# yc015/fully-automated-multi-heartbeat-echocardiography-video-segmentation-and-motion-tracking

Hardware: AMD Instinct MI355X
Metric: 32f×112×112 clips/sec at 1/2/4/8 MI355X; Dice Δ vs CPU ref (higher is better)
Workload: dtype fp32

## Files before the change

### fully-automated-multi-heartbeat-echocardiography-video-segmentation-and-motion-tracking_amd/_lib.py

```python
import ctypes
import os

from .build import LIB_PATH

c_int, c_int64, c_void_p, c_char_p = ctypes.c_int, ctypes.c_int64, ctypes.c_void_p, ctypes.c_char_p
_P = c_void_p

SIGNATURES = {
    "clasfv_last_error": (c_char_p, []),
    "clasfv_version": (c_int, []),
    "clasfv_source_hash": (c_char_p, []),
    "clasfv_create": (c_int, [c_int, ctypes.POINTER(c_void_p)]),
    "clasfv_destroy": (c_int, [_P]),
    "clasfv_param_count": (c_int, [_P]),
    "clasfv_param_info": (c_int, [_P, c_int, ctypes.POINTER(c_char_p), ctypes.POINTER(c_int), ctypes.POINTER(c_int64)]),
    "clasfv_load_param": (c_int, [_P, c_char_p, _P, c_int64]),
    "clasfv_finalize": (c_int, [_P]),
    "clasfv_forward": (c_int, [_P, _P, c_int, c_int, c_int, c_int, _P, _P, _P]),
    "clasfv_workspace_bytes": (c_int64, [_P]),
    "clasfv_set_compute_dtype": (c_int, [_P, c_int]),
    "clasfv_get_compute_dtype": (c_int, [_P]),
    "clasfv_set_kernel_variants": (c_int, [_P, c_int]),
    "clasfv_get_kernel_variants": (c_int, [_P]),
    "clasfv_set_kernel_timing": (c_int, [_P, c_int]),
    "clasfv_kernel_timing": (c_int, [_P, c_int, ctypes.POINTER(c_char_p), ctypes.POINTER(c_int),
                                     ctypes.POINTER(ctypes.c_double), ctypes.POINTER(ctypes.c_double),
                                     ctypes.POINTER(ctypes.c_double)]),
    "clasfv_set_launch_log": (c_int, [_P, c_int]),
    "clasfv_launch_log": (c_int, [_P, c_int, ctypes.POINTER(c_char_p), ctypes.POINTER(c_int64), ctypes.POINTER(c_int),
                                  ctypes.POINTER(c_int)]),
    "clasfv_fill_workspace": (c_int, [_P, c_int, _P]),
    "clasfv_conv_count": (c_int, [_P]),
    "clasfv_conv_info": (c_int, [_P, c_int, ctypes.POINTER(c_char_p), ctypes.POINTER(c_char_p), ctypes.POINTER(c_int),
                                 ctypes.POINTER(c_int), ctypes.POINTER(c_int), ctypes.POINTER(c_int),
                                 ctypes.POINTER(c_int), ctypes.POINTER(c_int), ctypes.POINTER(c_int)]),
    "clasfv_run_conv": (c_int, [_P, c_int, _P, c_int, c_int, c_int, c_int, _P, _P, c_int, c_int, c_int, _P, _P, c_int64,
                                ctypes.POINTER(c_char_p), _P]),
    "clasfv_run_decoder": (c_int, [_P, _P, _P, _P, _P, c_int, c_int, c_int, c_int, _P, _P, _P]),
    "clasfv_build_clips": (c_int, [_P, c_int, c_int, c_int, _P, c_int, c_int, _P, _P]),
    "clasfv_pass_labels": (c_int, [_P, c_int, _P, c_int, c_int, c_int, c_int, c_int, _P, _P]),
    "clasfv_pass_labels_margin": (c_int, [_P, c_int, _P, c_int, c_int, c_int, c_int, c_int, _P, _P]),
    "clasfv_logit_margin": (c_int, [_P, c_int, c_int, c_int, _P, _P]),
    "clasfv_fuse_votes": (c_int, [_P, c_int, c_int, c_int, c_int, c_int, c_int, _P, _P]),
    "clasfv_warp": (c_int, [_P, c_int, c_int, c_int, c_int, _P, c_int64, c_int64, _P, _P]),
    "clasfv_zeroone_workspace_bytes": (c_int64, []),
    "clasfv_zeroone_normalize": (c_int, [_P, c_int64, _P, _P]),
    "clasfv_warp_backward": (c_int, [_P, _P, c_int, c_int, c_int, c_int, _P, c_int64, c_int64, _P, _P, _P]),
    "clasfv_preprocess_video": (c_int, [_P, c_int, c_int, c_int, c_int, c_int, _P, _P]),
    "clasfv_track": (c_int, [_P, c_int, c_int, c_int, c_int, _P, c_int64, c_int64, c_int64, c_int, c_int, c_int, c_int,
                             c_int, _P, _P]),
    "clasfv_lv_geometry": (c_int, [_P, c_int64, c_int, c_int, c_int, ctypes.c_double, ctypes.c_double, _P, _P, _P]),
}

ABI_VERSION = 3
FUSE_MAJORITY, FUSE_SIMPLE, FUSE_STAPLE, FUSE_ITKVOTING = 0, 1, 2, 3
FUSE_FORCE_GENERIC = 0x100
TRACK_BILINEAR, TRACK_NEAREST = 0, 1
TRACK_FORCE_STEPS, TRACK_FORCE_LDS = 0x100, 0x200
TRACK_LDS_MAX_PIXELS, TRACK_LDS_AUTO_PIXELS = 20480, 2304
LV_NPUCKS, LV_STRIDE, LV_MAX_PIXELS = 10, 12, 162816
VARIANTS = {"no_winograd": 1, "no_wino_patch": 2, "winot_reference": 4, "no_c8": 8, "no_stem_bf16": 16,
            "no_patch_bf16": 32, "no_decoder_bf16": 64, "winot_no_ts1": 128, "no_split_k": 256, "no_wino4": 512,
            "no_decoder_x3": 1024, "no_dma_x3": 2048, "no_stem_x3": 4096, "no_wino4w": 8192,
            "no_patch32": 16384, "no_proj_x3": 32768, "no_wino4r": 65536,
            "no_dma_buf": 262144, "w4r_cached_stores": 524288,
            "patch32_cached_stores": 4194304, "no_dma_w": 16777216, "no_twalk": 67108864}
DTYPES = {"fp32": 0, "float32": 0, "bf16": 1, "bfloat16": 1}
_lib = None


def lib_path():
    return LIB_PATH


def load():
    global _lib
    if _lib is not None:
        return _lib
    from . import build as B
    want = B.source_hash()
    have = B.library_hash()
    if have != want:
        import sys
        print(f"clasfv: {LIB_PATH} {'missing' if have is None and not os.path.exists(LIB_PATH) else 'stale'} "
              f"(library source hash {have}, sources {want}): rebuilding", file=sys.stderr)
        B.build()
        if B.library_hash() != want:
            raise RuntimeError(f"{LIB_PATH}: rebuild did not produce a library of the current sources")
    lib = ctypes.CDLL(LIB_PATH)
    for name, (res, args) in SIGNATURES.items():
        fn = getattr(lib, name)
        fn.restype = res
        fn.argtypes = args
    if lib.clasfv_version() != ABI_VERSION:
        raise RuntimeError(f"{LIB_PATH}: ABI version {lib.clasfv_version()}, expected {ABI_VERSION}: rebuild it "
                           f"(python -m clasfv_amd.build --force)")
    got = lib.clasfv_source_hash().decode()
    if got != B.HASH_MARK.decode() + want:
        raise RuntimeError(f"{LIB_PATH}: loaded library reports {got}, sources hash to {want}")
    _lib = lib
    return lib


def check(rc, what=""):
    if rc != 0:
        msg = load().clasfv_last_error()
        raise RuntimeError(f"{what} failed ({rc}): {msg.decode() if msg else ''}")
    return rc


def stream_ptr(stream=None, device=None):
    import torch
    s = stream if stream is not None else torch.cuda.current_stream(device)
    return ctypes.c_void_p(s.cuda_stream)


def ptr(t):
    return ctypes.c_void_p(t.data_ptr())
```

### fully-automated-multi-heartbeat-echocardiography-video-segmentation-and-motion-tracking_amd/build.py

```python
import hashlib
import os
import re
import shutil
import subprocess
import sys

PKG_DIR = os.path.dirname(os.path.abspath(__file__))
REPO_DIR = os.path.dirname(PKG_DIR)
CSRC = os.path.join(PKG_DIR, "csrc")
INCLUDE = os.path.join(REPO_DIR, "include")
LIB_PATH = os.path.join(PKG_DIR, "libclasfv.so")
SOURCES = ["engine.hip", "conv.hip", "conv_patch.hip", "winograd.hip", "winograd2.hip", "winograd4.hip", "winograd4w.hip",
           "winograd_t.hip", "decoder.hip", "plumbing.hip", "twalk.hip", "track.hip", "lvgeom.hip"]
HEADERS = ["common.h", "lvgeom.h", "plumbing.h", "track.h", "warp_math.h", "wino4_common.h"]
ARCH = os.environ.get("CLASFV_OFFLOAD_ARCH", "gfx950")
EXTRA_FLAGS = {"winograd_t.hip": ["-fno-slp-vectorize"]}


def _hipcc():
    for c in (os.environ.get("HIPCC"), "/opt/rocm/bin/hipcc", shutil.which("hipcc")):
        if c and os.path.exists(c):
            return c
    raise RuntimeError("hipcc not found: the CLAS-FV engine needs ROCm's hipcc to build libclasfv.so")


def _inputs():
    files = [os.path.join(CSRC, f) for f in SOURCES + HEADERS]
    files.append(os.path.join(INCLUDE, "clasfv.h"))
    return files


HASH_MARK = b"clasfv-source-hash:"


def source_hash():
    h = hashlib.sha256()
    h.update(repr((ARCH, sorted(EXTRA_FLAGS.items()))).encode())
    for f in _inputs():
        h.update(os.path.basename(f).encode() + b"\0")
        with open(f, "rb") as fh:
            h.update(fh.read())
    return h.hexdigest()[:16]


def library_hash(path=LIB_PATH):
    if not os.path.exists(path):
        return None
    with open(path, "rb") as fh:
        m = re.search(re.escape(HASH_MARK) + rb"([0-9a-f]{16})", fh.read())
    return m.group(1).decode() if m else None


def up_to_date():
    return library_hash() == source_hash()


def build(force=False, verbose=False):
    if not force and up_to_date():
        return LIB_PATH
    import fcntl
    with open(os.path.join(PKG_DIR, "build.lock"), "w") as lock:
        fcntl.flock(lock, fcntl.LOCK_EX)
        if not force and up_to_date():
            return LIB_PATH
        return _build_locked(verbose)


def _build_locked(verbose):
    import tempfile
    from concurrent.futures import ThreadPoolExecutor
    os.makedirs(os.path.join(PKG_DIR, "build_obj"), exist_ok=True)
    objdir = tempfile.mkdtemp(prefix="build-", dir=os.path.join(PKG_DIR, "build_obj"))
    hipcc = _hipcc()
    flags = [f"--offload-arch={ARCH}", "-O3", "-std=c++17", "-fPIC", "-I", INCLUDE]
    digest = source_hash()

    def compile_one(src):
        obj = os.path.join(objdir, os.path.splitext(src)[0] + ".o")
        extra = list(EXTRA_FLAGS.get(src, []))
        if src == "engine.hip":
            extra.append(f'-DCLASFV_SOURCE_HASH="{digest}"')
        cmd = [hipcc] + flags + extra + ["-c", os.path.join(CSRC, src), "-o", obj]
        if verbose:
            print(" ".join(cmd), file=sys.stderr)
        r = subprocess.run(cmd, cwd=CSRC, capture_output=True, text=True)
        if r.returncode != 0:
            raise RuntimeError(f"hipcc failed on {src} ({r.returncode}):\n{r.stderr[-6000:]}")
        return obj

    jobs = max(1, min(len(SOURCES), int(os.environ.get("MAX_JOBS", os.cpu_count() or 4))))
    try:
        with ThreadPoolExecutor(jobs) as ex:
            objs = list(ex.map(compile_one, SOURCES))
        tmp = os.path.join(objdir, "libclasfv.so")
        r = subprocess.run([hipcc, f"--offload-arch={ARCH}", "-shared", "-fPIC", "-o", tmp] + objs,
                           capture_output=True, text=True)
        if r.returncode != 0:
            raise RuntimeError(f"link failed ({r.returncode}):\n{r.stderr[-6000:]}")
        os.replace(tmp, LIB_PATH)
    finally:
        shutil.rmtree(objdir, ignore_errors=True)
    return LIB_PATH


if __name__ == "__main__":
    print(build(force="--force" in sys.argv, verbose=True))
```

### fully-automated-multi-heartbeat-echocardiography-video-segmentation-and-motion-tracking_amd/csrc/common.h

```cpp
#pragma once
#include <hip/hip_runtime.h>
#include <stdint.h>

#include "clasfv.h"

typedef float f32x4 __attribute__((ext_vector_type(4)));
typedef float f32x2 __attribute__((ext_vector_type(2)));

__device__ inline float relu1(float x) { return __int_as_float(max(__float_as_int(x), 0)); }

__device__ inline f32x4 psub4(f32x4 a, f32x4 b) {
  const f32x2 alo = {a[0], a[1]}, ahi = {a[2], a[3]}, blo = {b[0], b[1]}, bhi = {b[2], b[3]};
  f32x2 lo, hi;
  asm("v_pk_add_f32 %0, %1, %2 neg_lo:[0,1] neg_hi:[0,1]" : "=v"(lo) : "v"(alo), "v"(blo));
  asm("v_pk_add_f32 %0, %1, %2 neg_lo:[0,1] neg_hi:[0,1]" : "=v"(hi) : "v"(ahi), "v"(bhi));
  return f32x4{lo[0], lo[1], hi[0], hi[1]};
}


struct FastDiv {
  unsigned m;
  int l;
};
inline FastDiv fast_div(unsigned d) {
  int l = 0;
  while ((1u << l) < d) ++l;
  return FastDiv{(unsigned)(((1ull << 32) * ((1ull << l) - d)) / d + 1), l};
}
__device__ inline int fdiv(int n, FastDiv f) { return (int)((__umulhi((unsigned)n, f.m) + (unsigned)n) >> f.l); }

struct LaunchNote {
  const void* kernel;
  long grid;
  int passes;
};
struct LaunchRing {
  unsigned n;
  LaunchNote e[4];
};
inline thread_local LaunchRing g_launch_ring;
inline void note_launch(const void* kernel, dim3 grid, long passes) {
  LaunchRing& r = g_launch_ring;
  r.e[r.n++ & 3] = LaunchNote{kernel, (long)grid.x * grid.y * grid.z, passes > 1 ? (int)passes : 1};
}
#define CLASFV_LAUNCH_P(passes, kernel, grid, ...)                       \
  do {                                                                   \
    const dim3 launch_grid_ = (grid);                                    \
    note_launch((const void*)(kernel), launch_grid_, (passes));          \
    hipLaunchKernelGGL(kernel, launch_grid_, __VA_ARGS__);               \
  } while (0)
#define CLASFV_LAUNCH(kernel, grid, ...) CLASFV_LAUNCH_P(1, kernel, grid, __VA_ARGS__)

struct ConvParams {
  const void* x;
  const void* w;
  const float* bias;
  const void* res;
  void* y;
  int N, Ti, Hi, Wi, Cin;
  int To, Ho, Wo, Cout;
  int KT, KH, KW, st, sh, sw, pt, ph, pw;
  int K, Kp, M, relu;
  const void* zero;
  const void* x2;
  int Cin2;
  int stem;
  int in_bf16, out_bf16;
  int x_c8, y_c8;
  int vflags, patch_nt;
  float* part;
  int n_split;
};

struct DecTap {
  const float* p;
  int T, H, W;
  float st, sh, sw;
};

struct DecParams {
  DecTap tap[4];
  const float* b1;
  const float* w2;
  const void* w2x3;
  const float* b2;
  const float* wh;
  const float* bh;
  float* seg;
  float* mot;
  int N, T, H, W;
  int bf16;
  int x3;
  void* idx;
};
inline size_t decoder_index_bytes(int T, int H, int W) { return (size_t)4 * (T + H + W) * 16; }

hipError_t launch_conv(const ConvParams& p, int mt, int bn, hipStream_t s);
void conv_pick_tile(int M, int cout_p, int force_nt, int* mt, int* bn);
bool wino_supported(const ConvParams& p);
hipError_t launch_wino(const ConvParams& p, hipStream_t s);
void wino_transform_weights(const double* w, int cout, int cin, int cout_p, int cin_p, float* U);
bool winoq_supported(const ConvParams& p);
hipError_t launch_winoq(const ConvParams& p, hipStream_t s);
bool wino4_supported(const ConvParams& p);
hipError_t launch_wino4(const ConvParams& p, hipStream_t s);
double wino4_exec_gflop(const ConvParams& p);
void wino4_transform_weights(const double* w, int cout, int cin, int cout_p, int cin_p, float* U);
size_t wino4_weight_floats(int cin_p, int cout_p);
bool wino4w_supported(const ConvParams& p);
hipError_t launch_wino4w(const ConvParams& p, hipStream_t s);
double wino4w_exec_gflop(const ConvParams& p);
void wino4w_transform_weights(const double* w, int cout, int cin, int cout_p, int cin_p, float* U);
size_t wino4w_weight_floats(int cin_p, int cout_p);
bool wino4r_supported(const ConvParams& p);
hipError_t launch_wino4r(const ConvParams& p, hipStream_t s);
double wino4r_exec_gflop(const ConvParams& p);
void wino4r_transform_weights(const double* w, int cout, int cin, int cout_p, int cin_p, float* U);
size_t wino4r_weight_floats(int cin_p, int cout_p);
bool winot_supported(const ConvParams& p);
hipError_t launch_winot(const ConvParams& p, hipStream_t s);
bool winot_c8_ok(const ConvParams& p);
hipError_t launch_split_sum(const ConvParams& p, hipStream_t s);
int dma_split_for(const ConvParams& p, int mt);
bool stem_x3_supported(const ConvParams& p);
hipError_t launch_stem_x3(const ConvParams& p, hipStream_t s);
bool dma_x3_supported(const ConvParams& p);
bool dma_w_ok(const ConvParams& p);
int dma_x3_bn(int cout_p);
hipError_t launch_dma_x3(const ConvParams& p, int bn, hipStream_t s);
void dma_x3_weight_image(const float* w, int cout_alloc, int Kp, uint16_t* out);
size_t dma_x3_weight_elems(int cout_alloc, int Kp);
int winot_split_for(const ConvParams& p);
void winot_transform_weights(const double* w, int cout, int cin, int cout_p, int cin_p, float* U);
bool proj_x3_supported(const ConvParams& p);
hipError_t launch_proj_x3(const ConvParams& p, hipStream_t s);
bool patch_bf16_supported(const ConvParams& p);
bool patch32_bf16_supported(const ConvParams& p);
hipError_t launch_patch32_bf16(const ConvParams& p, hipStream_t s);
hipError_t launch_patch_bf16(const ConvParams& p, hipStream_t s);
bool twalk_bf16_supported(const ConvParams& p);
hipError_t launch_twalk_bf16(const ConvParams& p, hipStream_t s);
bool stem_bf16_supported(const ConvParams& p);
hipError_t launch_stem_bf16(const ConvParams& p, hipStream_t s);
hipError_t launch_decoder(const DecParams& p, hipStream_t s);
constexpr int DECODER_X3_ELEMS = 3 * 4096 + 3 * 1024;
void decoder_x3_weights(const float* w2, const float* wh, uint16_t* out);
hipError_t launch_pack_input(const float* x, float* y, int N, int T, int HW, hipStream_t s);
```

### fully-automated-multi-heartbeat-echocardiography-video-segmentation-and-motion-tracking_amd/csrc/decoder.hip

```cpp
#include "common.h"

#include <string.h>

namespace {

constexpr int PIX = 72;
constexpr int TILE_W = 16;
template <int TH>
struct DecGeo {
  static constexpr int NTHR = 32 * TH;
  static constexpr int rows(int i) { return ((TH - 1) >> (i + 1)) + 3; }
  static constexpr int cols(int i) { return (15 >> (i + 1)) + 3; }
  static constexpr int kMaxRows[4] = {rows(0), rows(1), rows(2), rows(3)};
  static constexpr int kMaxCols[4] = {cols(0), cols(1), cols(2), cols(3)};
  static constexpr int kFrames[4] = {1, 2, 2, 2};
  static constexpr int kTapPix[4] = {rows(0) * cols(0), rows(1) * cols(1), rows(2) * cols(2), rows(3) * cols(3)};
  static constexpr int kPixOff[5] = {0, kTapPix[0], kTapPix[0] + kTapPix[1], kTapPix[0] + kTapPix[1] + kTapPix[2],
                                     kTapPix[0] + kTapPix[1] + kTapPix[2] + kTapPix[3]};
  static constexpr int STAGE_FLOATS = kPixOff[4] * PIX;
  static constexpr int ld(int i) { return (kTapPix[i] * 16 + NTHR - 1) / NTHR; }
  static constexpr int kLoads[4] = {ld(0), ld(1), ld(2), ld(3)};
  static constexpr int kLoadOff[4] = {0, ld(0), ld(0) + 2 * ld(1), ld(0) + 2 * ld(1) + 2 * ld(2)};
  static constexpr int kLoadsTotal = ld(0) + 2 * (ld(1) + ld(2) + ld(3));
  static constexpr int kLiveOff[5] = {0, ld(0), ld(0) + ld(1), ld(0) + ld(1) + ld(2), ld(0) + ld(1) + ld(2) + ld(3)};
// ... 189 lines not shown
        for (int mt = 0; mt < 2; ++mt)
          outs[mt] = __builtin_amdgcn_mfma_f32_16x16x4f32(wh[nt][r], acc[mt][nt][r], outs[mt], 0, 0, 0);
  }
#pragma unroll
  for (int mt = 0; mt < 2; ++mt) {
    const int hr = h0 + 2 * wid + mt;
    const f32x4 out = outs[mt];
    if (q < 2) {
      const size_t pix = (size_t)t * HW + (size_t)hr * p.W + (w0 + l16);
#pragma unroll
      for (int r = 0; r < 4; ++r) {
        const int co = 4 * q + r;
        if (co >= 6) continue;
        const float v = out[r];
        if (co < 2)
          p.seg[((size_t)n * 2 + co) * TH + pix] = v;
        else
          p.mot[((size_t)n * 4 + (co - 2)) * TH + pix] = fast_tanh(v);
      }
    }
  }
}

template <int MODE_, int TROWS = 8>
__global__ __launch_bounds__(32 * TROWS) __attribute__((amdgpu_waves_per_eu(((MODE_ & 7) == 4 && !(MODE_ & 64)) ? 4 : 5, ((MODE_ & 7) == 4 && !(MODE_ & 64)) ? 4 : 5))) void decoder_kernel(DecParams p) {
  constexpr int MODE = MODE_ & 7;
  constexpr bool SC = (MODE_ & 8) != 0;
  constexpr bool LIX = (MODE_ & 16) != 0;
  constexpr bool W2S = (MODE_ & 32) != 0;
  using G = DecGeo<TROWS>;
  constexpr int TILE_H = TROWS, NTHR = G::NTHR;
  constexpr int BF = MODE == 1 || MODE == 4;
  extern __shared__ __align__(16) float smem[];
  float* stage = smem;

  const int tid = threadIdx.x, lane = tid & 63;
  const int wid = __builtin_amdgcn_readfirstlane(tid >> 6);
  const int q = lane >> 4, l16 = lane & 15;
  const int tiles_w = p.W / TILE_W, tiles = (p.H / TILE_H) * tiles_w;
  int lt = xcd_swizzle_d(blockIdx.x, gridDim.x);
  const int tile = lt % tiles;
  lt /= tiles;
  const int t = lt % p.T, n = lt / p.T;
  const int h0 = (tile / tiles_w) * TILE_H, w0 = (tile % tiles_w) * TILE_W;


  const DecIdx* tab = reinterpret_cast<const DecIdx*>(p.idx);
  const int per = p.T + p.H + p.W;
  Win win[4];
#pragma unroll
  for (int i = 0; i < 4; ++i) {
    const DecTap& tp = p.tap[i];
    Win w;
    if constexpr (LIX) {
      int a, b;
      float la, lb;
      src_index(tp.st, t, tp.T, a, b, la, lb);
      const bool two = lb > 0.f && b != a && G::kFrames[i] == 2;
      w.t0 = uni(a);
      w.t1 = uni(two ? b : a);
      w.lt0 = unif(two ? la : 1.f);
      w.lt1 = unif(two ? lb : 0.f);
      const int r0 = min((int)floorf(tp.sh * (float)h0), tp.H - 1);
      const int r1 = min((int)floorf(tp.sh * (float)(h0 + TILE_H - 1)) + 1, tp.H - 1);
      const int c0 = min((int)floorf(tp.sw * (float)w0), tp.W - 1);
      const int c1 = min((int)floorf(tp.sw * (float)(w0 + TILE_W - 1)) + 1, tp.W - 1);
      w.r0 = uni(r0);
      w.nr = uni(min(r1 - r0 + 1, G::kMaxRows[i]));
      w.c0 = uni(c0);
      w.nc = uni(min(c1 - c0 + 1, G::kMaxCols[i]));
    } else {
      const DecIdx* ti = tab + i * per;
      const DecIdx ft = ti[t];
      w.t0 = ft.i0;
      w.t1 = ft.i1;
      w.lt0 = ft.l0;
      w.lt1 = ft.l1;
      const int r0 = ti[p.T + h0].i0, r1 = ti[p.T + h0 + TILE_H - 1].i1;
      const int c0 = ti[per - p.W + w0].i0, c1 = ti[per - p.W + w0 + TILE_W - 1].i1;
      w.r0 = r0;
      w.nr = min(r1 - r0 + 1, G::kMaxRows[i]);
      w.c0 = c0;
      w.nc = min(c1 - c0 + 1, G::kMaxCols[i]);
    }
    win[i] = w;
  }
  f32x4 buf[G::kLoadsTotal];
  bool live[G::kLiveOff[4]];
#pragma unroll
  for (int i = 0; i < 4; ++i) {
    const DecTap& tp = p.tap[i];
    const Win& w = win[i];
    const int base0 = (((n * tp.T + w.t0) * tp.H + w.r0) * tp.W + w.c0) * 64;
    const int base1 = base0 + (w.t1 - w.t0) * tp.H * tp.W * 64;
#pragma unroll
    for (int k = 0; k < G::kLoads[i]; ++k) {
      const int e = tid + NTHR * k;
      const int c4 = e & 15, px = e >> 4;
      const int rr = px / G::kMaxCols[i], cc = px - rr * G::kMaxCols[i];
      const bool lv = e < G::kTapPix[i] * 16 && rr < w.nr && cc < w.nc;
      live[G::kLiveOff[i] + k] = lv;
      const int lo = (rr * tp.W + cc) * 64 + c4 * 4;
#pragma unroll
      for (int f = 0; f < G::kFrames[i]; ++f) {
        f32x4& v = buf[G::kLoadOff[i] + k * G::kFrames[i] + f];
        if (lv) v = *reinterpret_cast<const f32x4*>(tp.p + (f ? base1 : base0) + lo);
      }
    }
  }
#pragma unroll
  for (int i = 0; i < 4; ++i) {
    const Win& w = win[i];
    float* dst = stage + G::kPixOff[i] * PIX;
#pragma unroll
    for (int k = 0; k < G::kLoads[i]; ++k) {
      const int e = tid + NTHR * k;
      if (live[G::kLiveOff[i] + k]) {
        f32x4 v = buf[G::kLoadOff[i] + k * G::kFrames[i]];
        if (G::kFrames[i] == 2) {
          const f32x4 v1 = buf[G::kLoadOff[i] + k * G::kFrames[i] + 1];
          if constexpr (SC) {
#pragma unroll
            for (int e = 0; e < 4; ++e) v[e] = fma1(v[e], w.lt0, mul1(v1[e], w.lt1));
          } else {
            v = v * w.lt0 + v1 * w.lt1;
          }
        }
        *reinterpret_cast<f32x4*>(dst + (e >> 4) * PIX + (e & 15) * 4) = v;
      }
    }
  }
  __syncthreads();

  const size_t HW = (size_t)p.H * p.W;
  const size_t TH = (size_t)p.T * HW;
  f32x4 h1[2][4];
#pragma unroll
  for (int mt = 0; mt < 2; ++mt)
#pragma unroll
    for (int c = 0; c < 4; ++c) h1[mt][c] = *reinterpret_cast<const f32x4*>(p.b1 + 16 * c + 4 * q);
  const int hr = h0 + 2 * wid;
#pragma unroll
  for (int i = 0; i < 4; ++i) {
    if constexpr (MODE == 3) {
#pragma unroll
      for (int c = 0; c < 4; ++c) h1[0][c] += *reinterpret_cast<const f32x4*>(stage + G::kPixOff[i] * PIX + 4 * q + 16 * c + l16 * PIX);
      continue;
    }
    const DecTap& tp = p.tap[i];
    const Win& w = win[i];
    int x0, x1, ya0, ya1, yb0, yb1;
    float lx0, lx1, la0, la1, lb0, lb1;
    if constexpr (LIX) {
      src_index(tp.sw, w0 + l16, tp.W, x0, x1, lx0, lx1);
      src_index(tp.sh, hr, tp.H, ya0, ya1, la0, la1);
      src_index(tp.sh, hr + 1, tp.H, yb0, yb1, lb0, lb1);
      ya0 = uni(ya0), ya1 = uni(ya1), yb0 = uni(yb0), yb1 = uni(yb1);
      la0 = unif(la0), la1 = unif(la1), lb0 = unif(lb0), lb1 = unif(lb1);
    } else {
      const DecIdx* ti = tab + i * per;
      const DecIdx cx = ti[per - p.W + w0 + l16];
      const DecIdx ra = ti[p.T + hr], rb = ti[p.T + hr + 1];
      x0 = cx.i0, x1 = cx.i1, lx0 = cx.l0, lx1 = cx.l1;
      ya0 = ra.i0, ya1 = ra.i1, la0 = ra.l0, la1 = ra.l1;
      yb0 = rb.i0, yb1 = rb.i1, lb0 = rb.l0, lb1 = rb.l1;
    }
    const int nrows = yb1 - ya0 + 1;
    const float* fb = stage + G::kPixOff[i] * PIX + 4 * q + (ya0 - w.r0) * G::kMaxCols[i] * PIX;
    const float* c0p = fb + (x0 - w.c0) * PIX;
    const float* c1p = fb + (x1 - w.c0) * PIX;
#pragma unroll
    for (int k = 0; k < 3; ++k) {
      if (k >= nrows) break;
      const bool ta = k == 0 || ya1 - ya0 == k, tb = yb0 - ya0 == k || yb1 - ya0 == k;
      const float wa = (k == 0 ? la0 : 0.f) + (ya1 - ya0 == k ? la1 : 0.f);
      const float wb = (yb0 - ya0 == k ? lb0 : 0.f) + (yb1 - ya0 == k ? lb1 : 0.f);
      const int ro = k * G::kMaxCols[i] * PIX;
      f32x4 hx[4];
      if constexpr (SC) {
#pragma unroll
        for (int c = 0; c < 4; ++c) {
          const f32x4 a0 = *reinterpret_cast<const f32x4*>(c0p + ro + 16 * c), a1 = *reinterpret_cast<const f32x4*>(c1p + ro + 16 * c);
#pragma unroll
          for (int e = 0; e < 4; ++e) hx[c][e] = fma1(a0[e], lx0, mul1(a1[e], lx1));
        }
        if (ta) {
#pragma unroll
          for (int c = 0; c < 4; ++c)
#pragma unroll
            for (int e = 0; e < 4; ++e) h1[0][c][e] = fma1(hx[c][e], wa, h1[0][c][e]);
        }
        if (tb) {
#pragma unroll
          for (int c = 0; c < 4; ++c)
#pragma unroll
            for (int e = 0; e < 4; ++e) h1[1][c][e] = fma1(hx[c][e], wb, h1[1][c][e]);
        }
      } else {
#pragma unroll
        for (int c = 0; c < 4; ++c)
          hx[c] = *reinterpret_cast<const f32x4*>(c0p + ro + 16 * c) * lx0 +
                  *reinterpret_cast<const f32x4*>(c1p + ro + 16 * c) * lx1;
        if (ta) {
#pragma unroll
          for (int c = 0; c < 4; ++c) h1[0][c] += hx[c] * wa;
        }
        if (tb) {
#pragma unroll
          for (int c = 0; c < 4; ++c) h1[1][c] += hx[c] * wb;
        }
      }
      __builtin_amdgcn_sched_barrier(0);
    }
  }
#pragma unroll
  for (int mt = 0; mt < 2; ++mt)
#pragma unroll
    for (int c = 0; c < 4; ++c)
#pragma unroll
      for (int j = 0; j < 4; ++j) h1[mt][c][j] = relu1(h1[mt][c][j]);

  if constexpr (BF) {
    decoder_heads_bf16<MODE == 4, true, W2S>(p, h1, t, n, h0, w0, wid, q, l16);
    return;
  }
  f32x4 acc[2][4], wa[4], wn[4];
#pragma unroll
  for (int c = 0; c < 4; ++c) wa[c] = *reinterpret_cast<const f32x4*>(p.w2 + l16 * 64 + 16 * c + 4 * q);
#pragma unroll
  for (int nt = 0; nt < 4; ++nt) {
    if (nt < 3) {
#pragma unroll
      for (int c = 0; c < 4; ++c)
        wn[c] = *reinterpret_cast<const f32x4*>(p.w2 + ((nt + 1) * 16 + l16) * 64 + 16 * c + 4 * q);
    }
    const f32x4 bb = *reinterpret_cast<const f32x4*>(p.b2 + 16 * nt + 4 * q);
    acc[0][nt] = bb;
    acc[1][nt] = bb;
    if constexpr (MODE == 2) {
#pragma unroll
      for (int mt = 0; mt < 2; ++mt) acc[mt][nt] += wa[nt] * h1[mt][nt];
    } else {
#pragma unroll
      for (int mt = 0; mt < 2; ++mt)
#pragma unroll
        for (int c = 0; c < 4; ++c)
#pragma unroll
          for (int j = 0; j < 4; ++j)
            acc[mt][nt] = __builtin_amdgcn_mfma_f32_16x16x4f32(wa[c][j], h1[mt][c][j], acc[mt][nt], 0, 0, 0);
    }
#pragma unroll
    for (int mt = 0; mt < 2; ++mt)
#pragma unroll
      for (int r = 0; r < 4; ++r) acc[mt][nt][r] = relu1(acc[mt][nt][r]);
#pragma unroll
    for (int c = 0; c < 4; ++c) wa[c] = wn[c];
  }
  f32x4 wh[4];
#pragma unroll
  for (int nt = 0; nt < 4; ++nt) {
    wh[nt] = *reinterpret_cast<const f32x4*>(p.wh + (l16 & 7) * 64 + 16 * nt + 4 * q);
    if (l16 >= 8) wh[nt] = f32x4{0.f, 0.f, 0.f, 0.f};
  }
  f32x4 hb;
#pragma unroll
  for (int r = 0; r < 4; ++r) hb[r] = 4 * q + r < 6 ? p.bh[4 * q + r] : 0.f;
  f32x4 outs[2] = {hb, hb};
  if constexpr (MODE == 2) {
#pragma unroll
    for (int mt = 0; mt < 2; ++mt)
#pragma unroll
      for (int nt = 0; nt < 4; ++nt) outs[mt] += wh[nt] * acc[mt][nt];
  } else {
#pragma unroll
    for (int nt = 0; nt < 4; ++nt)
#pragma unroll
      for (int r = 0; r < 4; ++r)
#pragma unroll
        for (int mt = 0; mt < 2; ++mt)
          outs[mt] = __builtin_amdgcn_mfma_f32_16x16x4f32(wh[nt][r], acc[mt][nt][r], outs[mt], 0, 0, 0);
  }
#pragma unroll
  for (int mt = 0; mt < 2; ++mt) {
    const int hr = h0 + 2 * wid + mt;
    const f32x4 out = outs[mt];
    if (q < 2) {
      const size_t pix = (size_t)t * HW + (size_t)hr * p.W + (w0 + l16);
#pragma unroll
      for (int r = 0; r < 4; ++r) {
        const int co = 4 * q + r;
        if (co >= 6) continue;
        const float v = out[r];
        if (co < 2)
          p.seg[((size_t)n * 2 + co) * TH + pix] = v;
        else
          p.mot[((size_t)n * 4 + (co - 2)) * TH + pix] = fast_tanh(v);
      }
    }
  }
}

}

static hipError_t launch_dec(const DecParams& p, hipStream_t s, int mode, int th = 8) {
  if (p.tap[0].T != p.T) return hipErrorInvalidValue;
  for (int i = 0; i < 4; ++i)
    if ((size_t)p.N * p.tap[i].T * p.tap[i].H * p.tap[i].W * 64 >= ((size_t)1 << 31)) return hipErrorInvalidValue;
  if (p.H % th || p.W % TILE_W) return hipErrorInvalidValue;
  const size_t nb = (size_t)(p.H / th) * (p.W / TILE_W) * p.T * p.N;
  if (nb >= ((size_t)1 << 31)) return hipErrorInvalidValue;
  static_assert(DecGeo<16>::STAGE_FLOATS * 4 <= 64 * 1024, "default dynamic LDS limit");
  const size_t lds = (size_t)(th == 16 ? DecGeo<16>::STAGE_FLOATS : DecGeo<8>::STAGE_FLOATS) * 4;
  void (*k)(DecParams) = nullptr;
  if (th == 8) k = mode == 1 ? decoder_kernel<1> : mode == 4 ? decoder_kernel<4> : mode == 0 ? decoder_kernel<0> : nullptr;
#ifdef CLASFV_KNOCKOUTS
  if (th == 16 && mode < 16) k = mode == 1 ? decoder_kernel<1, 16> : mode == 4 ? decoder_kernel<4, 16> : decoder_kernel<0, 16>;
  if (mode == 2) k = th == 16 ? decoder_kernel<2, 16> : decoder_kernel<2>;
  if (mode == 3) k = th == 16 ? decoder_kernel<3, 16> : decoder_kernel<3>;
  if (mode == 12) k = th == 16 ? decoder_kernel<12, 16> : decoder_kernel<12>;
  if (mode == 9) k = th == 16 ? decoder_kernel<9, 16> : decoder_kernel<9>;
  if (th == 8 && mode == 1 + 16 + 32) k = decoder_kernel<1 + 16 + 32>;
  if (th == 8 && mode == 4 + 16) k = decoder_kernel<4 + 16>;
  if (th == 8 && mode == 0 + 16) k = decoder_kernel<0 + 16>;
  if (th == 8 && mode == 1 + 16) k = decoder_kernel<1 + 16>;
  if (th == 8 && mode == 1 + 32) k = decoder_kernel<1 + 32>;
  if (th == 8 && mode == 4 + 64) k = decoder_kernel<4 + 64>;
#endif
  if (!k) return hipErrorInvalidValue;
  if (!(mode & 16)) {
    if (!p.idx) return hipErrorInvalidValue;
    const int ne = 4 * (p.T + p.H + p.W);
    CLASFV_LAUNCH(decoder_index_kernel, dim3((unsigned)((ne + 255) / 256)), dim3(256), 0, s, p);
  }
  CLASFV_LAUNCH(k, dim3((unsigned)nb), dim3(32 * th), lds, s, p);
  return hipGetLastError();
}

void decoder_x3_weights(const float* w2, const float* wh, uint16_t* out) {
  auto put = [&](double r, size_t i0, size_t stride) {
    for (int pc = 0; pc < 3; ++pc) {
      float f = (float)r;
      uint32_t u;
      memcpy(&u, &f, 4);
      const uint16_t b = (uint16_t)((u + 0x7fffu + ((u >> 16) & 1u)) >> 16);
      const uint32_t ub = (uint32_t)b << 16;
      float fb;
      memcpy(&fb, &ub, 4);
      out[i0 + pc * stride] = b;
      r -= fb;
    }
  };
  for (int nt = 0; nt < 4; ++nt)
    for (int kb = 0; kb < 2; ++kb)
      for (int l = 0; l < 16; ++l)
        for (int q = 0; q < 4; ++q)
          for (int e = 0; e < 8; ++e)
            put(w2[(16 * nt + l) * 64 + 32 * kb + 4 * q + (e < 4 ? e : 12 + e)],
                ((((size_t)nt * 2 + kb) * 16 + l) * 4 + q) * 8 + e, 4096);
  for (int kb = 0; kb < 2; ++kb)
    for (int l = 0; l < 16; ++l)
      for (int q = 0; q < 4; ++q)
        for (int e = 0; e < 8; ++e)
          put(l < 8 ? wh[l * 64 + 32 * kb + 4 * q + (e < 4 ? e : 12 + e)] : 0.0,
              3 * 4096 + (((size_t)kb * 16 + l) * 4 + q) * 8 + e, 1024);
}

hipError_t launch_decoder(const DecParams& p, hipStream_t s) {
  if ((p.x3 || p.bf16) && !p.w2x3) return hipErrorInvalidValue;
  const int mode = p.bf16 ? 1 : p.x3 ? 4 : 0;
  return launch_dec(p, s, mode, 8);
}

#ifdef CLASFV_KNOCKOUTS
hipError_t launch_decoder_ko(const DecParams& p, hipStream_t s, int ko) {
  const int m = ko & 15;
  const int base = m == 2 || m == 3 ? m : (p.bf16 ? 1 : p.x3 ? 4 : 0);
  int mode = (ko & 32) && (base == 1 || base == 4) ? base + 8 : base;
  if (ko & 64) mode += 16;
  if ((ko & 128) && base == 1) mode += 32;
  if ((ko & 256) && base == 4) mode += 64;
  return launch_dec(p, s, mode, (ko & 16) ? 16 : 8);
}
#endif
```

### fully-automated-multi-heartbeat-echocardiography-video-segmentation-and-motion-tracking_amd/csrc/engine.hip

```cpp
#include <cxxabi.h>
#include <math.h>
#include <stdio.h>
#include <stdlib.h>
#include <string.h>

#include <string>
#include <unordered_map>
#include <vector>

#include "clasfv.h"
#include "common.h"
#include "lvgeom.h"
#include "plumbing.h"
#include "track.h"

namespace {

thread_local std::string g_err;

int fail(int code, const std::string& msg) {
  g_err = msg;
  return code;
}

#define HIP_TRY(expr)                                                                        \
  do {                                                                                       \
    hipError_t _e = (expr);                                                                  \
    if (_e != hipSuccess) return fail(CLASFV_EHIP, std::string(#expr) + ": " + hipGetErrorString(_e)); \
  } while (0)

constexpr double kBnEps = 1e-5;

struct Param {
  std::string name;
  std::vector<int64_t> shape;
  std::vector<float> data;
  bool loaded = false;
  int64_t numel() const {
    int64_t n = 1;
    for (auto d : shape) n *= d;
    return n;
  }
};

int round_up(int x, int m) { return (x + m - 1) / m * m; }

int pad_channels(int c, bool bf16) {
  if (c == 3) return 4;
  const int step = bf16 ? 32 : 16;
  int cp = round_up(c, step);
  auto ok = [](int cp_) {
    for (int nt : {9, 8, 6, 5, 4, 3})
      if ((cp_ / 16) % nt == 0) return true;
    return false;
  };
  while (!ok(cp)) cp += step;
  return cp;
}

enum Role { STEM_S, STEM_T, SP1, TP1, SP2, TP2, DS, PROJ };

struct Conv {
  Role role;
  std::string w, bn;
  int cin, cout, cin_p, cout_p;
  int kt, kh, kw, st, sh, sw, pt, ph, pw;
  int K, Kp, cout_alloc;
  int cin2 = 0;
  int stem = 0, in_bf16 = 0, out_bf16 = 0;
  void* dw = nullptr;
  float* db = nullptr;
  void* dwino = nullptr;
  void* dwino4 = nullptr;
  void* dwino4w = nullptr;
  void* dwino4r = nullptr;
  void* dwinot = nullptr;
  void* dws16 = nullptr;
  void* dx3 = nullptr;
};

using ConvImage = void* Conv::*;
constexpr ConvImage kConvImages[] = {&Conv::dw,      &Conv::dwino,  &Conv::dwino4, &Conv::dwino4w,
                                     &Conv::dwino4r, &Conv::dwinot, &Conv::dws16,  &Conv::dx3};

void free_conv_images(Conv& c) {
  for (ConvImage img : kConvImages) {
    (void)hipFree(c.*img);
    c.*img = nullptr;
  }
  (void)hipFree(c.db);
  c.db = nullptr;
}

bool use_winot(const Conv& c, bool bf16, int vflags) {
  if (vflags & CLASFV_VARIANT_NO_WINOGRAD) return false;
  return !bf16 && (c.role == STEM_T || c.role == TP1 || c.role == TP2) && c.kt == 3 && c.kh == 1 && c.kw == 1 &&
         c.st == 1 && c.cin_p % 8 == 0 && c.cout_p % 64 == 0;
}

bool use_wino(const Conv& c, bool bf16, int vflags) {
  if (vflags & CLASFV_VARIANT_NO_WINOGRAD) return false;
  return !bf16 && (c.role == SP1 || c.role == SP2) && c.kt == 1 && c.kh == 3 && c.kw == 3 && c.sh == 1 &&
         c.sw == 1 && c.cin_p % 16 == 0 && c.cout_p % 48 == 0;
}

struct VariantSwitch {
  int bit;
  const char* env;
  bool zero_form;
};
constexpr VariantSwitch kVariants[] = {
    {CLASFV_VARIANT_NO_WINOGRAD, "CLASFV_WINOGRAD", true},
    {CLASFV_VARIANT_NO_WINO_PATCH, "CLASFV_NO_WINO_PATCH", false},
    {CLASFV_VARIANT_WINOT_REFERENCE, "CLASFV_WINOT_REFERENCE", false},
    {CLASFV_VARIANT_NO_C8, "CLASFV_NO_C8", false},
    {CLASFV_VARIANT_NO_STEM_BF16, "CLASFV_NO_STEM_BF16", false},
    {CLASFV_VARIANT_NO_PATCH_BF16, "CLASFV_NO_PATCH_BF16", false},
    {CLASFV_VARIANT_NO_DECODER_BF16, "CLASFV_NO_DECODER_BF16", false},
    {CLASFV_VARIANT_WINOT_NO_TS1, "CLASFV_WINOT_TS1", true},
    {CLASFV_VARIANT_NO_SPLIT_K, "CLASFV_NO_SPLIT_K", false},
    {CLASFV_VARIANT_NO_WINO4, "CLASFV_NO_WINO4", false},
    {CLASFV_VARIANT_NO_DECODER_X3, "CLASFV_NO_DECODER_X3", false},
    {CLASFV_VARIANT_NO_DMA_X3, "CLASFV_NO_DMA_X3", false},
    {CLASFV_VARIANT_NO_STEM_X3, "CLASFV_NO_STEM_X3", false},
    {CLASFV_VARIANT_NO_WINO4W, "CLASFV_NO_WINO4W", false},
    {CLASFV_VARIANT_NO_PATCH32, "CLASFV_NO_PATCH32", false},
    {CLASFV_VARIANT_NO_PROJ_X3, "CLASFV_NO_PROJ_X3", false},
    {CLASFV_VARIANT_NO_WINO4R, "CLASFV_NO_WINO4R", false},
    {CLASFV_VARIANT_NO_DMA_BUF, "CLASFV_NO_DMA_BUF", false},
    {CLASFV_VARIANT_W4R_CACHED_STORES, "CLASFV_W4R_CACHED_STORES", false},
    {CLASFV_VARIANT_PATCH32_CACHED_STORES, "CLASFV_PATCH32_CACHED_STORES", false},
    {CLASFV_VARIANT_NO_DMA_W, "CLASFV_NO_DMA_W", false},
    {CLASFV_VARIANT_NO_TWALK, "CLASFV_NO_TWALK", false},
};

int env_variants() {
  int f = 0;
  for (const VariantSwitch& v : kVariants) {
    const char* e = getenv(v.env);
    if (e && (!v.zero_form || e[0] == '0')) f |= v.bit;
  }
  return f;
}

constexpr int variant_mask() {
  int m = 0;
  for (const VariantSwitch& v : kVariants) m |= v.bit;
  return m;
}
constexpr int kVariantMask = variant_mask();

int env_int(const char* name) {
  const char* e = getenv(name);
  return e ? atoi(e) : 0;
}

void layout_conv(Conv& c, bool bf16) {
  c.stem = (c.role == STEM_S);
  c.in_bf16 = bf16 && !c.stem;
  c.out_bf16 = bf16 && c.role != PROJ;
  c.cin_p = pad_channels(c.cin, bf16);
  c.cout_p = c.role == PROJ ? c.cout : pad_channels(c.cout, bf16);
  c.K = c.kt * c.kh * c.kw * c.cin_p + c.cin2;
  c.Kp = round_up(c.K, c.in_bf16 ? 32 : 16);
  c.cout_alloc = c.cout_p;
}

Conv make_conv(Role role, const std::string& w, const std::string& bn, int cin, int cout, int kt, int kh, int kw,
               int st, int sh, int sw, int pt, int ph, int pw) {
  Conv c;
  c.role = role;
  c.w = w;
  c.bn = bn;
  c.cin = cin;
  c.cout = cout;
  c.kt = kt, c.kh = kh, c.kw = kw, c.st = st, c.sh = sh, c.sw = sw, c.pt = pt, c.ph = ph, c.pw = pw;
  layout_conv(c, false);
  return c;
}

int midplanes(int i, int o) { return (i * o * 27) / (i * 9 + 3 * o); }

struct Tuning {
  int vflags = 0, conv_nt = 0, patch_nt = 0;
};

}

struct clasfv_engine {
  int device = 0;
  std::vector<Param> params;
  std::unordered_map<std::string, int> index;
  std::vector<Conv> convs;
  Conv proj[5];
  float *b1 = nullptr, *w2 = nullptr, *b2 = nullptr, *wh = nullptr, *bh = nullptr;
  void* w2x3 = nullptr;
  bool ready = false;
  int dtype = CLASFV_DTYPE_FP32;
  Tuning tune;
  float* zero = nullptr;
  struct Ctx {
    hipStream_t stream = nullptr;
    char* arena = nullptr;
    size_t arena_bytes = 0;
    hipStream_t side = nullptr;
    hipEvent_t ev_fork = nullptr, ev_join = nullptr;
    uint64_t last_use = 0;
  };
  std::vector<Ctx*> ctxs;
  uint64_t ctx_clock = 0;
  bool ktime = false;
  std::vector<hipEvent_t> evs;
  int nev = 0;
  struct Rec {
    const char* name;
    double gflop;
    double xgflop;
    int e0, e1;
  };
  std::vector<Rec> recs;
  bool llog = false;
  struct LogRec {
    const char* label;
    long grid;
    int passes, conv;
  };
  std::vector<LogRec> log;
  std::unordered_map<const void*, std::string> labels;
};

namespace {

void add_param(clasfv_engine* e, const std::string& name, std::vector<int64_t> shape) {
  Param p;
  p.name = name;
  p.shape = std::move(shape);
  e->index[name] = (int)e->params.size();
  e->params.push_back(std::move(p));
}

void add_bn(clasfv_engine* e, const std::string& pre, int c) {
  add_param(e, pre + ".weight", {c});
  add_param(e, pre + ".bias", {c});
  add_param(e, pre + ".running_mean", {c});
  add_param(e, pre + ".running_var", {c});
  add_param(e, pre + ".num_batches_tracked", {});
}

void build_plan(clasfv_engine* e) {
  const std::string R = "r2plus1d_model.";
  auto reg = [&](const Conv& c) {
    add_param(e, c.w + ".weight", {c.cout, c.cin, c.kt, c.kh, c.kw});
    add_bn(e, c.bn, c.cout);
    e->convs.push_back(c);
  };
  reg(make_conv(STEM_S, R + "stem.0", R + "stem.1", 3, 45, 1, 7, 7, 1, 2, 2, 0, 3, 3));
  reg(make_conv(STEM_T, R + "stem.3", R + "stem.4", 45, 64, 3, 1, 1, 1, 1, 1, 1, 0, 0));
  int inplanes = 64;
  const int planes_l[4] = {64, 128, 256, 512}, stride_l[4] = {1, 2, 2, 2};
  for (int li = 0; li < 4; ++li) {
    const int planes = planes_l[li], stride = stride_l[li];
    for (int b = 0; b < 2; ++b) {
      const int st = b == 0 ? stride : 1;
      const int cin1 = b == 0 ? inplanes : planes;
      const int mid = midplanes(cin1, planes);
      const std::string pre = R + "layer" + std::to_string(li + 1) + "." + std::to_string(b) + ".";
      reg(make_conv(SP1, pre + "conv1.0.0", pre + "conv1.0.1", cin1, mid, 1, 3, 3, 1, st, st, 0, 1, 1));
      reg(make_conv(TP1, pre + "conv1.0.3", pre + "conv1.1", mid, planes, 3, 1, 1, st, 1, 1, 1, 0, 0));
      reg(make_conv(SP2, pre + "conv2.0.0", pre + "conv2.0.1", planes, mid, 1, 3, 3, 1, 1, 1, 0, 1, 1));
      reg(make_conv(TP2, pre + "conv2.0.3", pre + "conv2.1", mid, planes, 3, 1, 1, 1, 1, 1, 1, 0, 0));
      if (b == 0 && (stride != 1 || inplanes != planes))
        reg(make_conv(DS, pre + "downsample.0", pre + "downsample.1", inplanes, planes, 1, 1, 1, stride, stride,
                      stride, 0, 0, 0));
    }
    inplanes = planes;
  }
  add_param(e, R + "fc.weight", {400, 512});
  add_param(e, R + "fc.bias", {400});
  add_param(e, "comb_1_layer.weight", {64, 1024, 1, 1, 1});
  add_param(e, "comb_1_layer.bias", {64});
  add_bn(e, "comb_batch_norm_1", 64);
  add_param(e, "comb_2_layer.weight", {64, 64, 1, 1, 1});
  add_param(e, "comb_2_layer.bias", {64});
  add_bn(e, "comb_batch_norm_2", 64);
  add_param(e, "motion_head.weight", {4, 64, 1, 1, 1});
  add_param(e, "motion_head.bias", {4});
  add_param(e, "segmentation_head.weight", {2, 64, 1, 1, 1});
  add_param(e, "segmentation_head.bias", {2});
  const int tap_c[5] = {64, 64, 128, 256, 512};
  for (int i = 0; i < 5; ++i) e->proj[i] = make_conv(PROJ, "", "", tap_c[i], 64, 1, 1, 1, 1, 1, 1, 0, 0, 0);
  e->proj[0].cin2 = 64;
  layout_conv(e->proj[0], false);
}

const std::vector<float>& P(clasfv_engine* e, const std::string& n) { return e->params[e->index.at(n)].data; }

void bn_scale_shift(clasfv_engine* e, const std::string& bn, int c, std::vector<double>& s, std::vector<double>& t) {
  const auto& g = P(e, bn + ".weight");
  const auto& b = P(e, bn + ".bias");
  const auto& m = P(e, bn + ".running_mean");
  const auto& v = P(e, bn + ".running_var");
  s.resize(c);
  t.resize(c);
  for (int i = 0; i < c; ++i) {
    s[i] = (double)g[i] / sqrt((double)v[i] + kBnEps);
    t[i] = (double)b[i] - (double)m[i] * s[i];
  }
}

template <class T>
int upload(const std::vector<float>& h, T** d) {
  HIP_TRY(hipMalloc(d, h.size() * sizeof(float)));
  HIP_TRY(hipMemcpy(*d, h.data(), h.size() * sizeof(float), hipMemcpyHostToDevice));
  return CLASFV_OK;
}

uint16_t to_bf16(float f) {
  uint32_t u;
  memcpy(&u, &f, 4);
  u += 0x7FFF + ((u >> 16) & 1);
  return (uint16_t)(u >> 16);
}

int upload_bf16(const std::vector<float>& h, void** d) {
  std::vector<uint16_t> b(h.size());
  for (size_t i = 0; i < h.size(); ++i) b[i] = to_bf16(h[i]);
  HIP_TRY(hipMalloc(d, b.size() * sizeof(uint16_t)));
  HIP_TRY(hipMemcpy(*d, b.data(), b.size() * sizeof(uint16_t), hipMemcpyHostToDevice));
  return CLASFV_OK;
}

template <class F>
int upload_conv(Conv& c, F wsrc, const std::vector<double>& scale, const std::vector<double>& shift, bool has_bias) {
  std::vector<float> w((size_t)c.cout_alloc * c.Kp, 0.f);
  const int taps = c.kt * c.kh * c.kw;
  for (int o = 0; o < c.cout; ++o)
    for (int tap = 0; tap < taps; ++tap)
      for (int ci = 0; ci < c.cin; ++ci)
        w[(size_t)o * c.Kp + (size_t)tap * c.cin_p + ci] = (float)((double)wsrc(o, ci, tap) * scale[o]);
  int rc = c.in_bf16 ? upload_bf16(w, &c.dw) : upload(w, &c.dw);
  if (rc) return rc;
  if (!c.in_bf16 && !c.stem && c.Kp % 16 == 0) {
    std::vector<uint16_t> x3(dma_x3_weight_elems(c.cout_alloc, c.Kp));
    dma_x3_weight_image(w.data(), c.cout_alloc, c.Kp, x3.data());
    HIP_TRY(hipMalloc(&c.dx3, x3.size() * sizeof(uint16_t)));
    HIP_TRY(hipMemcpy(c.dx3, x3.data(), x3.size() * sizeof(uint16_t), hipMemcpyHostToDevice));
  }
  if (has_bias) {
    std::vector<float> b(c.cout_alloc, 0.f);
    for (int o = 0; o < c.cout; ++o) b[o] = (float)shift[o];
    rc = upload(b, &c.db);
  }
  return rc;
}

std::vector<double> folded_weights(const Conv& c, const std::vector<float>& w, const std::vector<double>& s, int taps) {
  const size_t per_o = (size_t)c.cin * taps;
  std::vector<double> wf((size_t)c.cout * per_o);
  for (int o = 0; o < c.cout; ++o)
    for (size_t i = 0; i < per_o; ++i) wf[o * per_o + i] = (double)w[o * per_o + i] * s[o];
  return wf;
}

int upload_wino_images(Conv& c, const std::vector<float>& w, const std::vector<double>& s) {
  const std::vector<double> wf = folded_weights(c, w, s, 9);
  int rc;
  std::vector<float> u((size_t)16 * c.cin_p * c.cout_p);
  wino_transform_weights(wf.data(), c.cout, c.cin, c.cout_p, c.cin_p, u.data());
  if ((rc = upload(u, &c.dwino))) return rc;
  if (c.cout_p % 48 == 0 && c.cin_p % 8 == 0) {
    std::vector<float> u4(wino4_weight_floats(c.cin_p, c.cout_p));
    wino4_transform_weights(wf.data(), c.cout, c.cin, c.cout_p, c.cin_p, u4.data());
    if ((rc = upload(u4, &c.dwino4))) return rc;
  }
  if (c.cin_p % 8 == 0 && wino4w_weight_floats(c.cin_p, c.cout_p)) {
    std::vector<float> uw(wino4w_weight_floats(c.cin_p, c.cout_p));
    wino4w_transform_weights(wf.data(), c.cout, c.cin, c.cout_p, c.cin_p, uw.data());
    if ((rc = upload(uw, &c.dwino4w))) return rc;
  }
  if (c.cin_p % 8 == 0 && wino4r_weight_floats(c.cin_p, c.cout_p)) {
    std::vector<float> ur(wino4r_weight_floats(c.cin_p, c.cout_p));
    wino4r_transform_weights(wf.data(), c.cout, c.cin, c.cout_p, c.cin_p, ur.data());
    if ((rc = upload(ur, &c.dwino4r))) return rc;
  }
  return CLASFV_OK;
}

int upload_winot_image(Conv& c, const std::vector<float>& w, const std::vector<double>& s) {
  const std::vector<double> wf = folded_weights(c, w, s, 3);
  std::vector<float> u((size_t)6 * c.cin_p * c.cout_p);
  winot_transform_weights(wf.data(), c.cout, c.cin, c.cout_p, c.cin_p, u.data());
  return upload(u, &c.dwinot);
}

template <class F>
void for_stem_taps(const Conv& c, const std::vector<float>& w, const std::vector<double>& s, F fn) {
  for (int o = 0; o < c.cout; ++o)
    for (int ci = 0; ci < c.cin; ++ci)
      for (int kh = 0; kh < 7; ++kh)
        for (int kw = 0; kw < 7; ++kw)
          fn((((size_t)o * 7 + kh) * 8 + kw) * 4 + ci, w[((size_t)o * c.cin + ci) * 49 + kh * 7 + kw], s[o]);
}

int upload_stem_images(Conv& c, const std::vector<float>& w, const std::vector<double>& s, bool bf16) {
  if (!c.stem || c.kh != 7 || c.kw != 7 || c.cin > 4) return CLASFV_OK;
  if (!bf16 && c.cout_p == 48) {
    const size_t img = (size_t)48 * 7 * 8 * 4;
    std::vector<float> ws(3 * img, 0.f);
    for_stem_taps(c, w, s, [&](size_t k, float wv, double scale) {
      double r = (double)(float)((double)wv * scale);
      for (int pc = 0; pc < 3; ++pc) {
        const uint32_t hb = (uint32_t)to_bf16((float)r) << 16;
        float f;
        memcpy(&f, &hb, 4);
        ws[pc * img + k] = f;
        r -= f;
      }
    });
    return upload_bf16(ws, &c.dws16);
  }
  if (bf16 && c.cout_p == 64) {
    const size_t img = (size_t)64 * 7 * 8 * 4;
    std::vector<float> ws(2 * img, 0.f);
    for_stem_taps(c, w, s, [&](size_t k, float wv, double scale) {
      const float v = (float)((double)wv * scale);
      const uint32_t hb = (uint32_t)to_bf16(v) << 16;
      float hi;
      memcpy(&hi, &hb, 4);
      ws[k] = hi;
      ws[img + k] = v - hi;
    });
    return upload_bf16(ws, &c.dws16);
  }
  return CLASFV_OK;
}

int finalize_conv(clasfv_engine* h, Conv& c, bool bf16) {
  free_conv_images(c);
  std::vector<double> s, t;
  bn_scale_shift(h, c.bn, c.cout, s, t);
  const auto& w = P(h, c.w + ".weight");
  const int taps = c.kt * c.kh * c.kw;
  const int cin = c.cin;
  int rc = upload_conv(
      c, [&](int o, int ci, int tap) { return w[((size_t)o * cin + ci) * taps + tap]; }, s, t, true);
  if (!rc && use_wino(c, bf16, h->tune.vflags)) rc = upload_wino_images(c, w, s);
  if (!rc) rc = upload_stem_images(c, w, s, bf16);
  if (!rc && use_winot(c, bf16, h->tune.vflags)) rc = upload_winot_image(c, w, s);
  return rc;
}

int finalize_projections(clasfv_engine* h) {
  std::vector<double> s, t;
  bn_scale_shift(h, "comb_batch_norm_1", 64, s, t);
  const auto& w1 = P(h, "comb_1_layer.weight");
  const std::vector<double> zero(64, 0.0);
  const int col0[5] = {0, 64, 128, 256, 512};
  for (int i = 0; i < 5; ++i) {
    if (i == 1) continue;
    Conv& c = h->proj[i];
    free_conv_images(c);
    const int o0 = col0[i];
    Conv tmp = c;
    tmp.cin = tmp.cin_p = c.cin + c.cin2;
    int rc = upload_conv(
        tmp, [&](int o, int ci, int) { return w1[(size_t)o * 1024 + o0 + ci]; }, s, zero, false);
    if (rc) return rc;
    c.dw = tmp.dw;
    c.dx3 = tmp.dx3;
  }
  return CLASFV_OK;
}

int finalize_decoder(clasfv_engine* h) {
  std::vector<double> s, t;
  bn_scale_shift(h, "comb_batch_norm_1", 64, s, t);
  const auto& bias1 = P(h, "comb_1_layer.bias");
  std::vector<float> b1(64);
  for (int o = 0; o < 64; ++o) b1[o] = (float)(s[o] * (double)bias1[o] + t[o]);
  bn_scale_shift(h, "comb_batch_norm_2", 64, s, t);
  const auto& w2 = P(h, "comb_2_layer.weight");
  const auto& bias2 = P(h, "comb_2_layer.bias");
  std::vector<float> w2f(64 * 64), b2(64);
  for (int o = 0; o < 64; ++o) {
    for (int k = 0; k < 64; ++k) w2f[o * 64 + k] = (float)((double)w2[o * 64 + k] * s[o]);
    b2[o] = (float)(s[o] * (double)bias2[o] + t[o]);
  }
  const auto& ws = P(h, "segmentation_head.weight");
  const auto& bs = P(h, "segmentation_head.bias");
  const auto& wm = P(h, "motion_head.weight");
  const auto& bm = P(h, "motion_head.bias");
  std::vector<float> whf(8 * 64, 0.f), bhf(8, 0.f);
  for (int k = 0; k < 64; ++k) {
    whf[0 * 64 + k] = ws[k];
    whf[1 * 64 + k] = ws[64 + k];
    for (int m = 0; m < 4; ++m) whf[(2 + m) * 64 + k] = wm[m * 64 + k];
  }
  bhf[0] = bs[0];
  bhf[1] = bs[1];
  for (int m = 0; m < 4; ++m) bhf[2 + m] = bm[m];
  for (float** d : {&h->b1, &h->w2, &h->b2, &h->wh, &h->bh}) {
    (void)hipFree(*d);
    *d = nullptr;
  }
  std::vector<uint16_t> w2x3(DECODER_X3_ELEMS);
  decoder_x3_weights(w2f.data(), whf.data(), w2x3.data());
  (void)hipFree(h->w2x3);
  h->w2x3 = nullptr;
  int rc = upload(b1, &h->b1);
  if (!rc) rc = upload(w2f, &h->w2);
// ... 36 lines not shown
}
double xg_stem_x3(const Conv&, const Shape5& out) {
  return 6 * 2.0 * ceil((double)out.n * out.t * out.h * out.w / 256.0) * 256.0 * 48.0 * 224.0 * 1e-9;
}
double xg_stem_bf16(const Conv&, const Shape5& out) {
  return 3 * 2.0 * ceil((double)out.n * out.t * out.h * out.w / 256.0) * 256.0 * 64.0 * 224.0 * 1e-9;
}
double xg_patch_bf16(const Conv& c, const Shape5& out) {
  const int fr = c.kt == 1 ? 2 : 4;
  const double px = c.kt == 1 ? (double)((out.h + 7) / 8 * 8) * ((out.w + 7) / 8 * 8)
                              : (double)((out.h * out.w + 63) / 64 * 64);
  return 2.0 * out.n * ((out.t + fr - 1) / fr * fr) * px * c.cout_p * (double)c.Kp * 1e-9;
}
double xg_proj_x3(const Conv& c, const Shape5& out) {
  return 6 * 2.0 * ceil((double)out.n * out.t * out.h * out.w / 32.0) * 32.0 * c.cout_p * (double)c.Kp * 1e-9;
}
double xg_twalk_bf16(const Conv& c, const Shape5& out) {
  return 2.0 * out.n * ((out.h * out.w + 31) / 32 * 32) * (double)c.cout_p * c.cin_p * (3.0 * out.t - 2.0) * 1e-9;
}
double xg_patch32_bf16(const Conv& c, const Shape5& out) {
  return 2.0 * out.n * ((out.t + 3) / 4 * 4) * (double)((out.h + 7) / 8 * 8) * ((out.w + 7) / 8 * 8) * c.cout_p *
         (double)c.Kp * 1e-9;
}
double xg_dma_x3(const Conv& c, const Shape5& out) {
  const double m = (double)out.n * out.t * out.h * out.w;
  return 6 * 2.0 * (ceil(m / 128.0) * 128.0) * c.cout_p * (double)((c.Kp + 31) / 32 * 32) * 1e-9;
}
double xg_gemm(const Conv& c, const Shape5& out) {
  const double m = (double)out.n * out.t * out.h * out.w;
  return 2.0 * (ceil(m / 128.0) * 128.0) * c.cout_p * (double)c.Kp * 1e-9;
}

enum Kernel {
  K_WINO4R, K_WINO4W, K_WINO4, K_WINO_Q, K_WINO, K_STEM_BF16, K_STEM_X3, K_WINOT, K_PATCH_BF16, K_PATCH32_BF16,
  K_TWALK_BF16, K_PROJ_X3, K_DMA_X3, K_STEM_F32, K_DMA_W, K_DMA
};

struct KernelInfo {
  Kernel id;
  const char* name;
  ConvImage image;
  bool writes_c8, reads_c8;
  double (*xgflop)(const Conv& c, const Shape5& out);
};
constexpr KernelInfo kKernels[] = {
    {K_WINO4R, "conv_wino4r", &Conv::dwino4r, true, false, xg_wino4r},
    {K_WINO4W, "conv_wino4w", &Conv::dwino4w, true, false, xg_wino4w},
    {K_WINO4, "conv_wino4", &Conv::dwino4, true, false, xg_wino4},
    {K_WINO_Q, "conv_wino_q", &Conv::dwino, true, false, xg_wino},
    {K_WINO, "conv_wino", &Conv::dwino, false, false, xg_wino},
    {K_STEM_BF16, "conv_stem_bf16", &Conv::dws16, false, false, xg_stem_bf16},
    {K_STEM_X3, "conv_stem_x3", &Conv::dws16, true, false, xg_stem_x3},
    {K_WINOT, "conv_winot", &Conv::dwinot, false, true, xg_winot},
    {K_PATCH_BF16, "conv_patch_bf16", &Conv::dw, false, false, xg_patch_bf16},
    {K_PATCH32_BF16, "conv_patch32_bf16", &Conv::dw, false, false, xg_patch32_bf16},
    {K_TWALK_BF16, "conv_twalk_bf16", &Conv::dw, false, false, xg_twalk_bf16},
    {K_PROJ_X3, "conv_proj_x3", &Conv::dx3, false, false, xg_proj_x3},
    {K_DMA_X3, "conv_dma_x3", &Conv::dx3, false, false, xg_dma_x3},
    {K_STEM_F32, "conv_stem_f32", &Conv::dw, true, false, xg_gemm},
    {K_DMA_W, "conv_dma_w", &Conv::dw, false, false, xg_gemm},
    {K_DMA, "conv_dma", &Conv::dw, false, false, xg_gemm},
};
constexpr bool kernels_in_order() {
  int i = 0;
  for (const KernelInfo& k : kKernels)
    if (k.id != i++) return false;
  return i == K_DMA + 1;
}
static_assert(kernels_in_order(), "kKernels: one row per Kernel enumerator, in the enum's order");

ConvParams conv_params(const Conv& c, const Shape5& in, Shape5& out) {
  out.n = in.n;
  out.t = (in.t + 2 * c.pt - c.kt) / c.st + 1;
  out.h = (in.h + 2 * c.ph - c.kh) / c.sh + 1;
  out.w = (in.w + 2 * c.pw - c.kw) / c.sw + 1;
  out.c = c.cout_p;
  ConvParams p{};
  p.w = c.dw;
  p.bias = c.db;
  p.N = in.n, p.Ti = in.t, p.Hi = in.h, p.Wi = in.w, p.Cin = in.c;
  p.To = out.t, p.Ho = out.h, p.Wo = out.w, p.Cout = out.c;
  p.KT = c.kt, p.KH = c.kh, p.KW = c.kw, p.st = c.st, p.sh = c.sh, p.sw = c.sw, p.pt = c.pt, p.ph = c.ph, p.pw = c.pw;
  p.K = c.K, p.Kp = c.Kp;
  p.M = out.n * out.t * out.h * out.w;
  p.Cin2 = c.cin2;
  p.stem = c.stem;
  p.in_bf16 = c.in_bf16;
  p.out_bf16 = c.out_bf16;
  return p;
}

Kernel pick_kernel(const Conv& c, ConvParams p) {
  if (c.dwino4 && c.dx3 && p.Ho * p.Wo <= 64 && !p.y_c8 && dma_x3_supported(p)) return K_DMA_X3;
  const int no4 = p.vflags & (CLASFV_VARIANT_NO_WINO4 | CLASFV_VARIANT_NO_WINO4W);
  if (c.dwino4r && !no4 && !(p.vflags & CLASFV_VARIANT_NO_WINO4R) && wino4r_supported(p)) return K_WINO4R;
  if (c.dwino4w && !no4 && wino4w_supported(p)) return K_WINO4W;
  if (c.dwino4 && !(p.vflags & CLASFV_VARIANT_NO_WINO4) && wino4_supported(p)) return K_WINO4;
  if (c.dwino) {
    const bool no_patch = (p.vflags & CLASFV_VARIANT_NO_WINO_PATCH) != 0;
    if (!no_patch && winoq_supported(p)) return K_WINO_Q;
    if (wino_supported(p)) return K_WINO;
  }
  if (c.dws16 && !(p.vflags & CLASFV_VARIANT_NO_STEM_BF16) && stem_bf16_supported(p)) return K_STEM_BF16;
  if (c.dws16 && stem_x3_supported(p)) return K_STEM_X3;
  if (c.dwinot && c.dx3 && (long)p.To * p.Ho * p.Wo <= 256 && !p.x_c8 && !p.y_c8 && dma_x3_supported(p))
    return K_DMA_X3;
  if (c.dwinot && winot_supported(p)) return K_WINOT;
  if (c.dx3 && !(p.vflags & CLASFV_VARIANT_NO_PROJ_X3) && proj_x3_supported(p)) return K_PROJ_X3;
  if (!(p.vflags & (CLASFV_VARIANT_NO_PATCH_BF16 | CLASFV_VARIANT_NO_PATCH32)) && patch32_bf16_supported(p))
    return K_PATCH32_BF16;
  if (!(p.vflags & (CLASFV_VARIANT_NO_PATCH_BF16 | CLASFV_VARIANT_NO_TWALK)) && twalk_bf16_supported(p))
    return K_TWALK_BF16;
  if (!(p.vflags & CLASFV_VARIANT_NO_PATCH_BF16) && patch_bf16_supported(p)) return K_PATCH_BF16;
  if (c.dx3 && dma_x3_supported(p)) return K_DMA_X3;
  if (c.stem) return K_STEM_F32;
  return dma_w_ok(p) ? K_DMA_W : K_DMA;
}

bool c8_pair(const Conv& a, const Conv& b, const Shape5& in, const Tuning& tu) {
  if (tu.vflags & CLASFV_VARIANT_NO_C8) return false;
  Shape5 mid, out;
  ConvParams pa = conv_params(a, in, mid);
  ConvParams pb = conv_params(b, mid, out);
  pa.vflags = pb.vflags = tu.vflags;
  return kKernels[pick_kernel(a, pa)].writes_c8 && !a.out_bf16 && kKernels[pick_kernel(b, pb)].reads_c8 &&
         winot_c8_ok(pb);
}

void split_k(ConvParams& p, int S, void* scratch, size_t scratch_bytes) {
  if (S > 1 && scratch && (size_t)S * p.M * p.Cout * sizeof(float) <= scratch_bytes) {
    p.part = reinterpret_cast<float*>(scratch);
    p.n_split = S;
  }
}

int run_conv(const Conv& c, const void* x, const Shape5& in, void* y, Shape5& out, const void* res, bool relu,
             hipStream_t s, const void* zero_block, const void* x2, const KernelInfo** kernel, const Tuning& tu,
             int x_c8 = 0, int y_c8 = 0, void* scratch = nullptr, size_t scratch_bytes = 0) {
  if (in.c != c.cin_p) return fail(CLASFV_EINVAL, "internal: channel mismatch");
  ConvParams p = conv_params(c, in, out);
  p.vflags = tu.vflags;
  p.patch_nt = tu.patch_nt;
  p.x = x;
  p.res = res;
  p.y = y;
  p.relu = relu ? 1 : 0;
  p.zero = zero_block;
  p.x2 = x2;
  p.x_c8 = x_c8;
  p.y_c8 = y_c8;
  const KernelInfo& k = kKernels[pick_kernel(c, p)];
  *kernel = &k;
  if ((y_c8 && !k.writes_c8) || (x_c8 && !k.reads_c8))
    return fail(CLASFV_EINVAL, "internal: 8-channel-blocked layout on an unsupported kernel");
  p.w = c.*k.image;
  switch (k.id) {
    case K_WINO4R: HIP_TRY(launch_wino4r(p, s)); break;
    case K_WINO4W: HIP_TRY(launch_wino4w(p, s)); break;
    case K_WINO4: HIP_TRY(launch_wino4(p, s)); break;
    case K_WINO_Q: HIP_TRY(launch_winoq(p, s)); break;
    case K_WINO: HIP_TRY(launch_wino(p, s)); break;
    case K_STEM_BF16: HIP_TRY(launch_stem_bf16(p, s)); break;
    case K_STEM_X3: HIP_TRY(launch_stem_x3(p, s)); break;
    case K_WINOT:
      split_k(p, winot_split_for(p), scratch, scratch_bytes);
      HIP_TRY(launch_winot(p, s));
      break;
    case K_PATCH_BF16: HIP_TRY(launch_patch_bf16(p, s)); break;
    case K_PATCH32_BF16: HIP_TRY(launch_patch32_bf16(p, s)); break;
    case K_TWALK_BF16: HIP_TRY(launch_twalk_bf16(p, s)); break;
    case K_PROJ_X3: HIP_TRY(launch_proj_x3(p, s)); break;
    case K_DMA_X3:
      split_k(p, dma_split_for(p, 2), scratch, scratch_bytes);
      HIP_TRY(launch_dma_x3(p, dma_x3_bn(c.cout_p), s));
      break;
    case K_STEM_F32:
      HIP_TRY(launch_conv(p, 2, c.cout_p, s));
      break;
    case K_DMA_W:
    case K_DMA: {
      int mt, bn;
      conv_pick_tile(p.M, c.cout_p, tu.conv_nt, &mt, &bn);
      split_k(p, dma_split_for(p, mt), scratch, scratch_bytes);
      HIP_TRY(launch_conv(p, mt, bn, s));
      break;
    }
  }
  return CLASFV_OK;
}

struct Layout {
  size_t off[32];
  size_t total;
};
enum Buf { XIN, S0, X0, MID, TA, DSB, L1A, L1, L2A, L2, L3A, L3, L4A, L4, P01, PP2, PP3, PP4, DIDX, NBUF };

void make_layout(int N, int T, int H, int W, Layout& L) {
  const size_t T1 = T, H2 = H / 2, W2 = W / 2;
  size_t sz[NBUF];
  sz[XIN] = (size_t)N * T * H * W * 4;
  sz[S0] = (size_t)N * T1 * H2 * W2 * 48;
  sz[X0] = (size_t)N * T1 * H2 * W2 * 64;
  const size_t l1 = (size_t)N * T1 * H2 * W2 * 64;
  const size_t l2 = (size_t)N * (T / 2) * (H / 4) * (W / 4) * 128;
  const size_t l3 = (size_t)N * (T / 4) * (H / 8) * (W / 8) * 256;
  const size_t l4 = (size_t)N * (T / 8) * (H / 16) * (W / 16) * 512;
  size_t mid = (size_t)N * T1 * H2 * W2 * 144;
  mid = std::max(mid, (size_t)N * T1 * (H / 4) * (W / 4) * 240);
  mid = std::max(mid, (size_t)N * (T / 2) * (H / 8) * (W / 8) * 480);
  mid = std::max(mid, (size_t)N * (T / 4) * (H / 16) * (W / 16) * 960);
  sz[MID] = mid;
  sz[TA] = std::max(std::max(l1, l2), std::max(l3, l4));
  sz[DSB] = std::max(l2, std::max(l3, l4));
  sz[L1A] = sz[L1] = l1;
  sz[L2A] = sz[L2] = l2;
  sz[L3A] = sz[L3] = l3;
  sz[L4A] = sz[L4] = l4;
  sz[P01] = (size_t)N * T1 * H2 * W2 * 64;
  sz[PP2] = (size_t)N * (T / 2) * (H / 4) * (W / 4) * 64;
  sz[PP3] = (size_t)N * (T / 4) * (H / 8) * (W / 8) * 64;
  sz[PP4] = (size_t)N * (T / 8) * (H / 16) * (W / 16) * 64;
  sz[DIDX] = decoder_index_bytes(T, H, W) / sizeof(float);
  size_t o = 0;
  for (int i = 0; i < NBUF; ++i) {
    L.off[i] = o;
    o += (sz[i] * sizeof(float) + 255) / 256 * 256;
  }
  L.total = o;
}

int tick(clasfv_engine* h, hipStream_t s) {
  if (h->nev == (int)h->evs.size()) {
    hipEvent_t e;
    if (hipEventCreate(&e) != hipSuccess) return -1;
    h->evs.push_back(e);
  }
  if (hipEventRecord(h->evs[h->nev], s) != hipSuccess) return -1;
  return h->nev++;
}

float tap_scale(int in, int out) { return out > 1 ? (float)(in - 1) / (float)(out - 1) : 0.f; }

DecParams decoder_params(const clasfv_engine* h, const float* const tap[4], const Shape5 tsh[4], float* seg, float* mot,
                         int N, int T, int H, int W, void* idx) {
  DecParams d{};
  for (int i = 0; i < 4; ++i) {
    d.tap[i].p = tap[i];
    d.tap[i].T = tsh[i].t;
    d.tap[i].H = tsh[i].h;
    d.tap[i].W = tsh[i].w;
    d.tap[i].st = tap_scale(tsh[i].t, T);
    d.tap[i].sh = tap_scale(tsh[i].h, H);
    d.tap[i].sw = tap_scale(tsh[i].w, W);
  }
  d.b1 = h->b1;
  d.w2 = h->w2;
  d.b2 = h->b2;
  d.wh = h->wh;
  d.bh = h->bh;
  d.seg = seg;
  d.mot = mot;
  d.N = N, d.T = T, d.H = H, d.W = W;
  d.bf16 = h->dtype == CLASFV_DTYPE_BF16 && !(h->tune.vflags & CLASFV_VARIANT_NO_DECODER_BF16);
  d.w2x3 = h->w2x3;
  d.x3 = h->dtype != CLASFV_DTYPE_BF16 && !(h->tune.vflags & CLASFV_VARIANT_NO_DECODER_X3);
  d.idx = idx;
  return d;
}

struct DeviceGuard {
  int prev = -1;
  hipError_t err = hipSuccess;
  explicit DeviceGuard(int dev) {
    err = hipGetDevice(&prev);
    if (err == hipSuccess && prev != dev) err = hipSetDevice(dev);
  }
  ~DeviceGuard() {
    int cur = -1;
    if (prev >= 0 && hipGetDevice(&cur) == hipSuccess && cur != prev) (void)hipSetDevice(prev);
  }
};

#define DEVICE_GUARD(dev)                                                                       \
  DeviceGuard _guard(dev);                                                                      \
  if (_guard.err != hipSuccess)                                                                 \
    return fail(CLASFV_EHIP, std::string("hipSetDevice: ") + hipGetErrorString(_guard.err))

int acquire_ctx(clasfv_engine* h, hipStream_t s, size_t bytes, clasfv_engine::Ctx** out) {
  clasfv_engine::Ctx* cx = nullptr;
  for (auto* c : h->ctxs)
    if (c->stream == s) cx = c;
  if (!cx) {
    constexpr size_t kMaxCtx = 4;
    if (h->ctxs.size() < kMaxCtx) {
      cx = new clasfv_engine::Ctx();
      h->ctxs.push_back(cx);
    } else {
      HIP_TRY(hipDeviceSynchronize());
      cx = h->ctxs.front();
      for (auto* c : h->ctxs)
        if (c->last_use < cx->last_use) cx = c;
    }
    cx->stream = s;
  }
  cx->last_use = ++h->ctx_clock;
  if (bytes > cx->arena_bytes) {
    HIP_TRY(hipDeviceSynchronize());
    (void)hipFree(cx->arena);
    cx->arena = nullptr;
    cx->arena_bytes = 0;
    HIP_TRY(hipMalloc(&cx->arena, bytes));
    cx->arena_bytes = bytes;
  }
  *out = cx;
  return CLASFV_OK;
}

const Conv* probe_conv(const clasfv_engine* h, int i, int* tap) {
  static const int kTap[4] = {0, 2, 3, 4};
  const int nb = (int)h->convs.size();
  if (i < 0 || i >= nb + 4) return nullptr;
  if (tap) *tap = i < nb ? -1 : kTap[i - nb];
  return i < nb ? &h->convs[i] : &h->proj[kTap[i - nb]];
}

int conv_index(const clasfv_engine* h, const Conv& c) {
  const int nb = (int)h->convs.size();
  if (&c >= h->convs.data() && &c < h->convs.data() + nb) return (int)(&c - h->convs.data());
  const int i = (int)(&c - h->proj);
  return nb + (i == 0 ? 0 : i - 1);
}

std::string label_of(const void* kernel) {
  const char* mangled = hipKernelNameRefByPtr(kernel, nullptr);
  if (!mangled) return "?";
  std::string m(mangled);
  for (size_t a; (a = m.find("DF16b")) != std::string::npos;) m.replace(a, 5, "Dh");
  int status = 0;
  char* d = abi::__cxa_demangle(m.c_str(), nullptr, nullptr, &status);
  std::string t(d && status == 0 ? d : mangled);
  free(d);
  for (size_t a; (a = t.find("half")) != std::string::npos;) t.replace(a, 4, "__bf16");
  const std::string anon = "(anonymous namespace)::";
  for (size_t a; (a = t.find(anon)) != std::string::npos;) t.erase(a, anon.size());
  if (t.compare(0, 5, "void ") == 0) t.erase(0, 5);
  const size_t lt = t.find('<'), par = t.find('(');
  if (lt != std::string::npos && lt < par) {
    int depth = 0;
    for (size_t i = lt; i < t.size(); ++i) {
      if (t[i] == '<') ++depth;
      if (t[i] == '>' && --depth == 0) return t.substr(0, i + 1);
    }
  }
  return t.substr(0, par);
}

constexpr size_t kMaxLog = 1 << 16;
void log_begin(const clasfv_engine* h) {
  if (h->llog) g_launch_ring.n = 0;
}
void log_end(clasfv_engine* h, int conv) {
  if (!h->llog) return;
  const LaunchRing& r = g_launch_ring;
  for (unsigned i = 0; i < r.n && i < 4 && h->log.size() < kMaxLog; ++i) {
    auto it = h->labels.find(r.e[i].kernel);
    if (it == h->labels.end()) it = h->labels.emplace(r.e[i].kernel, label_of(r.e[i].kernel)).first;
    h->log.push_back({it->second.c_str(), r.e[i].grid, r.e[i].passes, conv});
  }
}

}

extern "C" {

const char* clasfv_last_error(void) { return g_err.c_str(); }
int clasfv_version(void) { return CLASFV_ABI_VERSION; }
#ifndef CLASFV_SOURCE_HASH
#define CLASFV_SOURCE_HASH "unhashed"
#endif
const char* clasfv_source_hash(void) { return "clasfv-source-hash:" CLASFV_SOURCE_HASH; }

int clasfv_create(int device, clasfv_t* out) {
  if (!out) return fail(CLASFV_EINVAL, "null out");
  int n = 0;
  HIP_TRY(hipGetDeviceCount(&n));
  if (device < 0 || device >= n) return fail(CLASFV_EINVAL, "bad device index");
  auto* e = new clasfv_engine();
  e->device = device;
  e->tune.vflags = env_variants();
  e->tune.conv_nt = env_int("CLASFV_CONV_NT");
  e->tune.patch_nt = env_int("CLASFV_PATCH_NT");
  build_plan(e);
  *out = e;
  return CLASFV_OK;
}

int clasfv_destroy(clasfv_t h) {
  if (!h) return CLASFV_OK;
  DeviceGuard guard(h->device);
  for (auto& c : h->convs) free_conv_images(c);
  for (auto& c : h->proj) free_conv_images(c);
  for (auto* c : h->ctxs) {
    if (c->side) (void)hipStreamDestroy(c->side);
    if (c->ev_fork) (void)hipEventDestroy(c->ev_fork);
    if (c->ev_join) (void)hipEventDestroy(c->ev_join);
    (void)hipFree(c->arena);
    delete c;
  }
  (void)hipFree(h->b1);
  (void)hipFree(h->w2);
  (void)hipFree(h->w2x3);
  (void)hipFree(h->b2);
  (void)hipFree(h->wh);
  (void)hipFree(h->bh);
  (void)hipFree(h->zero);
  for (auto e : h->evs) (void)hipEventDestroy(e);
  delete h;
  return CLASFV_OK;
}

int clasfv_param_count(clasfv_t h) { return h ? (int)h->params.size() : CLASFV_EINVAL; }

int clasfv_param_info(clasfv_t h, int i, const char** name, int* ndim, int64_t dims[5]) {
  if (!h || i < 0 || i >= (int)h->params.size()) return fail(CLASFV_EINVAL, "bad param index");
  const Param& p = h->params[i];
  if (name) *name = p.name.c_str();
  if (ndim) *ndim = (int)p.shape.size();
  if (dims)
    for (size_t d = 0; d < p.shape.size(); ++d) dims[d] = p.shape[d];
  return CLASFV_OK;
}

int clasfv_load_param(clasfv_t h, const char* name, const float* data, int64_t numel) {
  if (!h || !name) return fail(CLASFV_EINVAL, "null argument");
  std::string n(name);
  if (n.rfind("module.", 0) == 0) n = n.substr(7);
  auto it = h->index.find(n);
  if (it == h->index.end()) return fail(CLASFV_EINVAL, "unknown parameter: " + n);
  Param& p = h->params[it->second];
  if (n.size() > 20 && n.compare(n.size() - 20, 20, ".num_batches_tracked") == 0) {
    p.loaded = true;
    return CLASFV_OK;
  }
  if (numel != p.numel()) return fail(CLASFV_EINVAL, "size mismatch for " + n);
  if (!data) return fail(CLASFV_EINVAL, "null data");
  p.data.assign(data, data + numel);
  p.loaded = true;
  h->ready = false;
  return CLASFV_OK;
}

int clasfv_finalize(clasfv_t h) {
  if (!h) return fail(CLASFV_EINVAL, "null handle");
  for (const auto& p : h->params)
    if (!p.loaded && p.name.find(".fc.") == std::string::npos)
      return fail(CLASFV_ENOTREADY, "parameter not loaded: " + p.name);
  DEVICE_GUARD(h->device);
  HIP_TRY(hipDeviceSynchronize());
  const bool bf16 = h->dtype == CLASFV_DTYPE_BF16;
  for (auto& c : h->convs) layout_conv(c, bf16);
  for (auto& c : h->proj) layout_conv(c, bf16);
  for (auto& c : h->convs)
    if (int rc = finalize_conv(h, c, bf16)) return rc;
  if (int rc = finalize_projections(h)) return rc;
  if (int rc = finalize_decoder(h)) return rc;
  if (!h->zero) {
    HIP_TRY(hipMalloc(&h->zero, 256));
    HIP_TRY(hipMemset(h->zero, 0, 256));
  }
  HIP_TRY(hipDeviceSynchronize());
  h->ready = true;
  return CLASFV_OK;
}

int64_t clasfv_workspace_bytes(clasfv_t h) {
  if (!h) return 0;
  int64_t b = 0;
  for (auto* c : h->ctxs) b += (int64_t)c->arena_bytes;
  return b;
}

int clasfv_set_compute_dtype(clasfv_t h, int dtype) {
  if (!h) return fail(CLASFV_EINVAL, "null handle");
  if (dtype != CLASFV_DTYPE_FP32 && dtype != CLASFV_DTYPE_BF16) return fail(CLASFV_EINVAL, "unknown dtype");
  if (dtype != h->dtype) {
    h->dtype = dtype;
    h->ready = false;
  }
  return CLASFV_OK;
}

int clasfv_get_compute_dtype(clasfv_t h) { return h ? h->dtype : CLASFV_EINVAL; }

int clasfv_set_kernel_variants(clasfv_t h, int flags) {
  if (!h) return fail(CLASFV_EINVAL, "null handle");
  if (flags & ~kVariantMask) return fail(CLASFV_EINVAL, "unknown kernel-variant bit");
  if ((flags ^ h->tune.vflags) & CLASFV_VARIANT_NO_WINOGRAD) h->ready = false;
  h->tune.vflags = flags;
  return CLASFV_OK;
}

int clasfv_get_kernel_variants(clasfv_t h) { return h ? h->tune.vflags : CLASFV_EINVAL; }

int clasfv_forward(clasfv_t h, const float* x, int N, int T, int H, int W, float* seg, float* mot, void* stream) {
  if (!h) return fail(CLASFV_EINVAL, "null handle");
  if (!h->ready) return fail(CLASFV_ENOTREADY, "clasfv_finalize has not been called");
  if (!x || !seg || !mot) return fail(CLASFV_EINVAL, "null tensor");
  if (N < 1) return fail(CLASFV_EINVAL, "N must be >= 1");
  if (T < 8 || H < 16 || W < 16 || T % 8 || H % 16 || W % 16)
    return fail(CLASFV_EBADSHAPE, "shape must satisfy T % 8 == 0, H % 16 == 0, W % 16 == 0 (got T=" +
                                      std::to_string(T) + " H=" + std::to_string(H) + " W=" + std::to_string(W) + ")");
  hipStream_t s = (hipStream_t)stream;
  DEVICE_GUARD(h->device);
  Layout L;
  make_layout(N, T, H, W, L);
  clasfv_engine::Ctx* cx = nullptr;
  if (int rc_ = acquire_ctx(h, s, L.total, &cx)) return rc_;
  char* const arena = cx->arena;
  auto buf = [&](int b) { return reinterpret_cast<void*>(arena + L.off[b]); };
  int last_ev = h->ktime ? tick(h, s) : -1;
  auto timed = [&](const char* name, double gflop, double xgflop) {
    if (last_ev < 0) return;
    const int e = tick(h, s);
    if (e >= 0) h->recs.push_back({name, gflop, xgflop, last_ev, e});
    last_ev = e;
  };
  const size_t mid_bytes = L.off[MID + 1] - L.off[MID];
  if (!cx->side) {
    HIP_TRY(hipStreamCreateWithFlags(&cx->side, hipStreamNonBlocking));
    HIP_TRY(hipEventCreateWithFlags(&cx->ev_fork, hipEventDisableTiming));
    HIP_TRY(hipEventCreateWithFlags(&cx->ev_join, hipEventDisableTiming));
  }
  struct SideJoin {
    clasfv_engine::Ctx* cx;
    hipStream_t s;
    bool pending = false;
    hipError_t join() {
      if (!pending) return hipSuccess;
      pending = false;
      hipError_t e = hipEventRecord(cx->ev_join, cx->side);
      return e != hipSuccess ? e : hipStreamWaitEvent(s, cx->ev_join, 0);
    }
    ~SideJoin() { (void)join(); }
  } side_join{cx, s};
  auto run_side = [&](const Conv& c, const void* xin, const Shape5& in, void* y, Shape5& out, const void* x2) {
    HIP_TRY(hipEventRecord(cx->ev_fork, s));
    HIP_TRY(hipStreamWaitEvent(cx->side, cx->ev_fork, 0));
    side_join.pending = true;
    const int e0 = h->ktime ? tick(h, cx->side) : -1;
    const KernelInfo* k = nullptr;
    log_begin(h);
    int rc_ = run_conv(c, xin, in, y, out, nullptr, false, cx->side, h->zero, x2, &k, h->tune);
    log_end(h, conv_index(h, c));
    if (!rc_ && e0 >= 0) {
      const int e1 = tick(h, cx->side);
      if (e1 >= 0) h->recs.push_back({k->name, conv_gflop(c, out), k->xgflop(c, out), e0, e1});
    }
    return rc_;
  };
  auto run = [&](const Conv& c, const void* xin, const Shape5& in, void* y, Shape5& out, const void* res, bool relu,
                 const void* x2 = nullptr, int x_c8 = 0, int y_c8 = 0) {
    const KernelInfo* k = nullptr;
    void* scratch = nullptr;
    size_t scratch_bytes = 0;
    if (xin == buf(MID)) {
      const size_t used = ((size_t)in.n * in.t * in.h * in.w * in.c * sizeof(float) + 255) / 256 * 256;
      if (used < mid_bytes) {
        scratch = arena + L.off[MID] + used;
        scratch_bytes = mid_bytes - used;
      }
    }
    log_begin(h);
    int rc_ = run_conv(c, xin, in, y, out, res, relu, s, h->zero, x2, &k, h->tune, x_c8, y_c8, scratch, scratch_bytes);
    log_end(h, conv_index(h, c));
    if (!rc_) timed(k->name, conv_gflop(c, out), k->xgflop(c, out));
    return rc_;
  };

  log_begin(h);
  HIP_TRY(launch_pack_input(x, reinterpret_cast<float*>(buf(XIN)), N, T, H * W, s));
  log_end(h, -1);
  timed("pack_input_kernel", 0.0, 0.0);
  Shape5 sx{N, T, H, W, 4}, s0, sx0;
  Shape5 sp, sp2, sp3, sp4;
  int rc;
  size_t ci = 0;
  const int c8s = c8_pair(h->convs[0], h->convs[1], sx, h->tune);
  if ((rc = run(h->convs[ci++], buf(XIN), sx, buf(S0), s0, nullptr, true, nullptr, 0, c8s))) return rc;
  if ((rc = run(h->convs[ci++], buf(S0), s0, buf(X0), sx0, nullptr, true, nullptr, c8s, 0))) return rc;
  const int outs[4][2] = {{L1A, L1}, {L2A, L2}, {L3A, L3}, {L4A, L4}};
  void* cur = buf(X0);
  Shape5 cs = sx0, taps_shape[5];
  void* taps[5];
  taps[0] = cur;
  taps_shape[0] = cs;
  for (int li = 0; li < 4; ++li) {
    for (int b = 0; b < 2; ++b) {
      const Conv& sp1 = h->convs[ci++];
      const Conv& tp1 = h->convs[ci++];
      const Conv& sp2 = h->convs[ci++];
      const Conv& tp2 = h->convs[ci++];
      const Conv* ds = (ci < h->convs.size() && h->convs[ci].role == DS) ? &h->convs[ci++] : nullptr;
      Shape5 sm, sa, sm2, so, sd;
      const int c8a = c8_pair(sp1, tp1, cs, h->tune);
      if ((rc = run(sp1, cur, cs, buf(MID), sm, nullptr, true, nullptr, 0, c8a))) return rc;
      if ((rc = run(tp1, buf(MID), sm, buf(TA), sa, nullptr, true, nullptr, c8a, 0))) return rc;
      const int c8b = c8_pair(sp2, tp2, sa, h->tune);
      if ((rc = run(sp2, buf(TA), sa, buf(MID), sm2, nullptr, true, nullptr, 0, c8b))) return rc;
      const void* res = cur;
      if (ds) {
        if ((rc = run(*ds, cur, cs, buf(DSB), sd, nullptr, false))) return rc;
        res = buf(DSB);
      }
      void* out = buf(outs[li][b]);
      if ((rc = run(tp2, buf(MID), sm2, out, so, res, true, nullptr, c8b, 0))) return rc;
      cur = out;
      cs = so;
    }
    taps[li + 1] = cur;
    taps_shape[li + 1] = cs;
    if (li == 2) {
      if ((rc = run_side(h->proj[0], taps[0], taps_shape[0], buf(P01), sp, taps[1]))) return rc;
      if ((rc = run_side(h->proj[2], taps[2], taps_shape[2], buf(PP2), sp2, nullptr))) return rc;
      if ((rc = run_side(h->proj[3], taps[3], taps_shape[3], buf(PP3), sp3, nullptr))) return rc;
    }
  }
  if ((rc = run(h->proj[4], taps[4], taps_shape[4], buf(PP4), sp4, nullptr, false))) return rc;
  HIP_TRY(side_join.join());

  const Shape5 tsh[4] = {sp, sp2, sp3, sp4};
  const int tb[4] = {P01, PP2, PP3, PP4};
  const float* tp[4];
  for (int i = 0; i < 4; ++i) tp[i] = reinterpret_cast<const float*>(buf(tb[i]));
  const DecParams d = decoder_params(h, tp, tsh, seg, mot, N, T, H, W, buf(DIDX));
  log_begin(h);
  HIP_TRY(launch_decoder(d, s));
  log_end(h, -1);
  const double dec_px = d.x3 ? 6.0 * (64 * 64 + 64 * 16) : d.bf16 ? 3.0 * 64 * 64 + 6.0 * 64 * 16 : 64 * 64 + 64 * 16;
  timed(d.x3 || d.bf16 ? "decoder_kernel" : "decoder_kernel_f32", 2.0 * N * (double)T * H * W * (64 * 64 + 64 * 6) * 1e-9,
        2.0 * N * (double)T * H * W * dec_px * 1e-9);
  return CLASFV_OK;
}

int clasfv_set_kernel_timing(clasfv_t h, int enable) {
  if (!h) return fail(CLASFV_EINVAL, "null handle");
  h->ktime = enable != 0;
  h->recs.clear();
  h->nev = 0;
  return CLASFV_OK;
}

int clasfv_kernel_timing(clasfv_t h, int cap, const char** names, int* launches, double* ms, double* gflop,
                         double* xgflop) {
  if (!h || cap < 0 || (cap > 0 && (!names || !launches || !ms || !gflop || !xgflop)))
    return fail(CLASFV_EINVAL, "bad argument");
  if (h->nev > 0) HIP_TRY(hipEventSynchronize(h->evs[h->nev - 1]));
  int n = 0;
  for (const auto& r : h->recs) {
    float t = 0.f;
    HIP_TRY(hipEventElapsedTime(&t, h->evs[r.e0], h->evs[r.e1]));
    int i = 0;
    while (i < n && strcmp(names[i], r.name) != 0) ++i;
    if (i == n) {
      if (n == cap) return fail(CLASFV_EINVAL, "kernel timing: cap too small");
      names[n] = r.name;
      launches[n] = 0;
      ms[n] = gflop[n] = xgflop[n] = 0.0;
      ++n;
    }
    launches[i] += 1;
    ms[i] += t;
    gflop[i] += r.gflop;
    xgflop[i] += r.xgflop;
  }
  h->recs.clear();
  h->nev = 0;
  return n;
}

int clasfv_set_launch_log(clasfv_t h, int enable) {
  if (!h) return fail(CLASFV_EINVAL, "null handle");
  h->llog = enable != 0;
  h->log.clear();
  return CLASFV_OK;
}

int clasfv_launch_log(clasfv_t h, int cap, const char** labels, int64_t* grids, int* passes, int* convs) {
  if (!h) return fail(CLASFV_EINVAL, "null handle");
  if (cap < 0 || (cap > 0 && (!labels || !grids || !passes || !convs))) return fail(CLASFV_EINVAL, "bad argument");
  if (h->log.size() > (size_t)cap) return fail(CLASFV_EINVAL, "launch log: cap too small");
  const int n = (int)h->log.size();
  for (int i = 0; i < n; ++i) {
    labels[i] = h->log[i].label;
    grids[i] = h->log[i].grid;
    passes[i] = h->log[i].passes;
    convs[i] = h->log[i].conv;
  }
  h->log.clear();
  return n;
}

int clasfv_fill_workspace(clasfv_t h, int byte, void* stream) {
  if (!h) return fail(CLASFV_EINVAL, "null handle");
  if (byte < 0 || byte > 255) return fail(CLASFV_EINVAL, "fill byte must be in [0, 255]");
  hipStream_t s = (hipStream_t)stream;
  clasfv_engine::Ctx* cx = nullptr;
  for (auto* c : h->ctxs)
    if (c->stream == s) cx = c;
  if (!cx || !cx->arena) return fail(CLASFV_EINVAL, "no workspace exists for this stream yet");
  DEVICE_GUARD(h->device);
  HIP_TRY(hipMemsetAsync(cx->arena, byte, cx->arena_bytes, s));
  return CLASFV_OK;
}


int clasfv_conv_count(clasfv_t h) { return h ? (int)h->convs.size() + 4 : CLASFV_EINVAL; }

int clasfv_conv_info(clasfv_t h, int i, const char** prefix, const char** bn_prefix, int* tap, int channels[5],
                     int kernel[3], int stride[3], int padding[3], int* in_dtype, int* out_dtype) {
  if (!h) return fail(CLASFV_EINVAL, "null handle");
  int tp = -1;
  const Conv* pc = probe_conv(h, i, &tp);
  if (!pc) return fail(CLASFV_EINVAL, "bad conv index");
  Conv c = *pc;
  layout_conv(c, h->dtype == CLASFV_DTYPE_BF16);
  if (prefix) *prefix = pc->w.c_str();
  if (bn_prefix) *bn_prefix = pc->bn.c_str();
  if (tap) *tap = tp;
  if (channels) channels[0] = c.cin, channels[1] = c.cout, channels[2] = c.cin_p, channels[3] = c.cout_p, channels[4] = c.cin2;
  if (kernel) kernel[0] = c.kt, kernel[1] = c.kh, kernel[2] = c.kw;
  if (stride) stride[0] = c.st, stride[1] = c.sh, stride[2] = c.sw;
  if (padding) padding[0] = c.pt, padding[1] = c.ph, padding[2] = c.pw;
  if (in_dtype) *in_dtype = c.in_bf16 ? CLASFV_DTYPE_BF16 : CLASFV_DTYPE_FP32;
  if (out_dtype) *out_dtype = c.out_bf16 ? CLASFV_DTYPE_BF16 : CLASFV_DTYPE_FP32;
  return CLASFV_OK;
}

int clasfv_run_conv(clasfv_t h, int i, const void* x, int N, int T, int H, int W, const void* x2, const void* res,
                    int relu, int x_c8, int y_c8, void* y, void* scratch, int64_t scratch_bytes,
                    const char** kernel_name, void* stream) {
  if (!h) return fail(CLASFV_EINVAL, "null handle");
  if (!h->ready) return fail(CLASFV_ENOTREADY, "clasfv_finalize has not been called");
  const Conv* c = probe_conv(h, i, nullptr);
  if (!c) return fail(CLASFV_EINVAL, "bad conv index");
  if (!x || !y) return fail(CLASFV_EINVAL, "null tensor");
  if (N < 1 || T < 1 || H < 1 || W < 1) return fail(CLASFV_EINVAL, "bad shape");
  if ((c->cin2 != 0) != (x2 != nullptr)) return fail(CLASFV_EINVAL, "second input: needed by the dual projection only");
  if (scratch_bytes < 0 || (scratch_bytes > 0 && !scratch)) return fail(CLASFV_EINVAL, "bad scratch");
  if (T + 2 * c->pt < c->kt || H + 2 * c->ph < c->kh || W + 2 * c->pw < c->kw)
    return fail(CLASFV_EINVAL, "input smaller than the kernel");
  DEVICE_GUARD(h->device);
  const Shape5 in{N, T, H, W, c->cin_p};
  Shape5 out;
  const KernelInfo* k = nullptr;
  log_begin(h);
  int rc = run_conv(*c, x, in, y, out, res, relu != 0, (hipStream_t)stream, h->zero, x2, &k, h->tune, x_c8, y_c8,
                    scratch_bytes ? scratch : nullptr, (size_t)scratch_bytes);
  log_end(h, i);
  if (kernel_name) *kernel_name = k ? k->name : "";
  return rc;
}

int clasfv_run_decoder(clasfv_t h, const float* p01, const float* p2, const float* p3, const float* p4, int N, int T,
                       int H, int W, float* seg, float* mot, void* stream) {
  if (!h) return fail(CLASFV_EINVAL, "null handle");
  if (!h->ready) return fail(CLASFV_ENOTREADY, "clasfv_finalize has not been called");
  if (!p01 || !p2 || !p3 || !p4 || !seg || !mot) return fail(CLASFV_EINVAL, "null tensor");
  if (N < 1 || T < 1 || H < 2 || W < 2) return fail(CLASFV_EINVAL, "bad shape");
  if (H % 8 || W % 16) return fail(CLASFV_EBADSHAPE, "decoder tiles: H % 8 == 0 and W % 16 == 0");
  hipStream_t s = (hipStream_t)stream;
  DEVICE_GUARD(h->device);
  Layout L;
  make_layout(N, T, H, W, L);
  clasfv_engine::Ctx* cx = nullptr;
  if (int rc = acquire_ctx(h, s, L.total, &cx)) return rc;
  auto half = [](int d) { return (d - 1) / 2 + 1; };
  const float* taps[4] = {p01, p2, p3, p4};
  Shape5 tsh[4];
  int t = T, hh = half(H), ww = half(W);
  for (int k = 0; k < 4; ++k) {
    if (k) t = half(t), hh = half(hh), ww = half(ww);
    tsh[k] = Shape5{N, t, hh, ww, 64};
  }
  log_begin(h);
  HIP_TRY(launch_decoder(decoder_params(h, taps, tsh, seg, mot, N, T, H, W, cx->arena + L.off[DIDX]), s));
  log_end(h, -1);
  return CLASFV_OK;
}

int clasfv_build_clips(const float* video, int T, int H, int W, const int32_t* table, int n, int interp, float* clips,
                       void* stream) {
  if (!video || !table || !clips || n < 0 || T < 1 || H < 1 || W < 1) return fail(CLASFV_EINVAL, "bad argument");
  if (n == 0) return CLASFV_OK;
  HIP_TRY(launch_build_clips(video, T, H * W, table, n, interp, clips, (hipStream_t)stream));
  return CLASFV_OK;
}

static int check_pass_labels(const void* in, int K, const int32_t* clip0, int T, int step, int H, int W, int interp,
                             const void* labels) {
  if (!in || !clip0 || !labels || K < 1 || K > CLASFV_MAX_PASSES || T < 1 || step < 1)
    return fail(CLASFV_EINVAL, "bad argument (K must be in [1, 64])");
  if (H < 1 || W < 1) return fail(CLASFV_EINVAL, "bad argument (H and W must be >= 1)");
  if (T > 65535) return fail(CLASFV_EINVAL, "bad argument (T must be <= 65535)");
  if ((int64_t)(K - 1) * step >= T) return fail(CLASFV_EINVAL, "bad argument ((K - 1) * step must be < T)");
  for (int k = 0; k < K; ++k) {
    const int tk = T - k * step;
    const int q = tk >> 5, r = tk & 31;
    const int nk = r > 16 ? q + 1 : r < 16 ? q : q + (q & 1);
    if (nk == 0) return fail(CLASFV_EINVAL, "a pass has too few frames for one 32-frame clip");
    if (clip0[k] < 0) return fail(CLASFV_EINVAL, "negative pass_clip0 entry");
    if (!interp && r != 0) return fail(CLASFV_EINVAL, "interpolate == 0 needs every pass length to be a multiple of 32");
  }
  return CLASFV_OK;
}

int clasfv_pass_labels(const float* logits, int K, const int32_t* clip0, int T, int step, int H, int W, int interp,
                       uint8_t* labels, void* stream) {
  if (int rc = check_pass_labels(logits, K, clip0, T, step, H, W, interp, labels)) return rc;
  HIP_TRY(launch_pass_labels(logits, K, clip0, T, step, H * W, interp, 0, labels, (hipStream_t)stream));
  return CLASFV_OK;
}

int clasfv_pass_labels_margin(const float* margin, int K, const int32_t* clip0, int T, int step, int H, int W,
                              int interp, uint8_t* labels, void* stream) {
  if (int rc = check_pass_labels(margin, K, clip0, T, step, H, W, interp, labels)) return rc;
  HIP_TRY(launch_pass_labels(margin, K, clip0, T, step, H * W, interp, 1, labels, (hipStream_t)stream));
  return CLASFV_OK;
}

int clasfv_logit_margin(const float* logits, int n, int H, int W, float* margin, void* stream) {
  if (!logits || !margin || n < 0 || H < 1 || W < 1) return fail(CLASFV_EINVAL, "bad argument");
  if (n == 0) return CLASFV_OK;
  HIP_TRY(launch_logit_margin(logits, n, H * W, margin, (hipStream_t)stream));
  return CLASFV_OK;
}

int clasfv_fuse_votes(const uint8_t* labels, int K, int T, int step, int H, int W, int method, uint8_t* fused,
                      void* stream) {
  if (!labels || !fused || K < 1 || K > CLASFV_MAX_PASSES || T < 1 || step < 1 || T - (step - 1) < 1)
    return fail(CLASFV_EINVAL, "bad argument (K must be in [1, 64])");
  const int m = method & ~CLASFV_FUSE_FORCE_GENERIC;
  if (m != CLASFV_FUSE_MAJORITY && m != CLASFV_FUSE_SIMPLE && m != CLASFV_FUSE_STAPLE && m != CLASFV_FUSE_ITKVOTING)
    return fail(CLASFV_EINVAL, "unknown method");
  if (H < 1 || W < 1) return fail(CLASFV_EINVAL, "bad argument (H and W must be >= 1)");
  if ((m == CLASFV_FUSE_MAJORITY || m == CLASFV_FUSE_ITKVOTING) && T - (step - 1) > 65535)
    return fail(CLASFV_EINVAL, "bad argument (majority / ITK voting take at most 65535 output frames)");
  if (m == CLASFV_FUSE_SIMPLE && (int64_t)H * W > CLASFV_SIMPLE_MAX_HW)
    return fail(CLASFV_EBADSHAPE, "SIMPLE keeps one frame's estimate in LDS: H * W must be <= 162816");
  HIP_TRY(launch_fuse_votes(labels, K, T, step, H * W, method, fused, (hipStream_t)stream));
  return CLASFV_OK;
}

int clasfv_warp(const float* img, int N, int C, int H, int W, const float* motion, int64_t m_sn, int64_t m_sc,
                float* out, void* stream) {
  if (!img || !motion || !out || N < 1 || C < 1 || H < 1 || W < 1) return fail(CLASFV_EINVAL, "bad argument");
  HIP_TRY(launch_warp(img, N, C, H, W, motion, m_sn, m_sc, out, (hipStream_t)stream));
  return CLASFV_OK;
}

int clasfv_warp_backward(const float* grad_out, const float* img, int N, int C, int H, int W, const float* motion,
                         int64_t m_sn, int64_t m_sc, float* grad_img, float* grad_motion, void* stream) {
  if (!grad_out || !img || !motion || (!grad_img && !grad_motion) || N < 1 || C < 1 || H < 1 || W < 1)
    return fail(CLASFV_EINVAL, "bad argument");
  HIP_TRY(launch_warp_backward(grad_out, img, N, C, H, W, motion, m_sn, m_sc, grad_img, grad_motion,
                               (hipStream_t)stream));
  return CLASFV_OK;
}

int clasfv_track(const float* img, int N, int C, int H, int W, const float* motion, int64_t m_sn, int64_t m_sc,
                 int64_t m_st, int T, int t0, int t_step, int P, int mode, float* out, void* stream) {
  if (!img || !motion || !out) return fail(CLASFV_EINVAL, "bad argument (null pointer)");
  if (N < 1 || C < 1 || H < 1 || W < 1) return fail(CLASFV_EINVAL, "bad argument (N, C, H and W must be >= 1)");
  if (P < 1) return fail(CLASFV_EINVAL, "bad argument (P must be >= 1)");
  if (t_step != 1 && t_step != -1) return fail(CLASFV_EINVAL, "bad argument (t_step must be +1 or -1)");
  const int64_t t_last = t0 + (int64_t)(P - 1) * t_step;
  if (T < 1 || t0 < 0 || t0 >= T || t_last < 0 || t_last >= T)
    return fail(CLASFV_EINVAL, "bad argument (every frame t0 + p * t_step, p < P, must lie in [0, T))");
  const int both = CLASFV_TRACK_FORCE_STEPS | CLASFV_TRACK_FORCE_LDS, m = mode & ~both;
  if ((m != CLASFV_TRACK_BILINEAR && m != CLASFV_TRACK_NEAREST) || (mode & both) == both)
    return fail(CLASFV_EINVAL, "unknown mode");
  if ((int64_t)H * W > INT32_MAX || (int64_t)N * C > INT32_MAX)
    return fail(CLASFV_EBADSHAPE, "H * W and N * C must be < 2^31");
  const uintptr_t i0 = (uintptr_t)img, o0 = (uintptr_t)out;
  const uint64_t frame = (uint64_t)N * C * H * W * sizeof(float);
  if (i0 < o0 + frame * (uint64_t)P && o0 < i0 + frame) return fail(CLASFV_EINVAL, "out overlaps img");
  HIP_TRY(launch_track(img, N, C, H, W, motion, m_sn, m_sc, m_st, t0, t_step, P, mode, out, (hipStream_t)stream));
  return CLASFV_OK;
}

int clasfv_lv_geometry(const uint8_t* masks, int64_t F, int H, int W, int label, double sy, double sx, int32_t* area,
                       double* geom, void* stream) {
  if (!masks || !area || !geom) return fail(CLASFV_EINVAL, "bad argument (null pointer)");
  if (F < 1 || H < 1 || W < 1) return fail(CLASFV_EINVAL, "bad argument (F, H and W must be >= 1)");
  if (label < 0 || label > 255) return fail(CLASFV_EINVAL, "bad argument (label must be in [0, 255])");
  if (!(isfinite(sy) && isfinite(sx) && sy > 0.0 && sx > 0.0))
    return fail(CLASFV_EINVAL, "bad argument (the spacings must be finite and positive)");
  if ((int64_t)H * W > CLASFV_LV_MAX_PIXELS)
    return fail(CLASFV_EBADSHAPE, "the frame is kept in LDS: H * W must be <= 162816");
  HIP_TRY(launch_lv_geometry(masks, F, H, W, label, sy, sx, area, geom, (hipStream_t)stream));
  return CLASFV_OK;
}

int clasfv_preprocess_video(const uint8_t* frames, int T, int Hs, int Ws, int H, int W, float* out, void* stream) {
  if (!frames || !out || T < 1 || Hs < 1 || Ws < 1 || H < 1 || W < 1 || H > 65535 || T > 65535)
    return fail(CLASFV_EINVAL, "bad argument");
  HIP_TRY(launch_preprocess_video(frames, T, Hs, Ws, H, W, out, (hipStream_t)stream));
  return CLASFV_OK;
}

int64_t clasfv_zeroone_workspace_bytes(void) { return (int64_t)sizeof(float) * zeroone_partials_floats(); }

int clasfv_zeroone_normalize(float* video, int64_t n, float* workspace, void* stream) {
  if (!video || !workspace || n < 1) return fail(CLASFV_EINVAL, "bad argument");
  HIP_TRY(launch_zeroone_normalize(video, n, workspace, (hipStream_t)stream));
  return CLASFV_OK;
}

}
```

### fully-automated-multi-heartbeat-echocardiography-video-segmentation-and-motion-tracking_amd/csrc/plumbing.h

```cpp
#pragma once
#include <hip/hip_runtime.h>
#include <stdint.h>

#define CLASFV_MAX_PASSES 64
#define CLASFV_SIMPLE_MAX_HW (160 * 1024 - 1024)

hipError_t launch_build_clips(const float* video, int T, int HW, const int32_t* table, int n, int interp, float* clips,
                              hipStream_t s);
hipError_t launch_pass_labels(const float* logits, int K, const int32_t* clip0, int T, int step, int HW, int interp,
                              int margin, uint8_t* labels, hipStream_t s);
hipError_t launch_logit_margin(const float* logits, int n, int HW, float* margin, hipStream_t s);
hipError_t launch_fuse_votes(const uint8_t* labels, int K, int T, int step, int HW, int method, uint8_t* fused,
                             hipStream_t s);
hipError_t launch_warp(const float* img, int N, int C, int H, int W, const float* motion, int64_t m_sn, int64_t m_sc,
                       float* out, hipStream_t s);
hipError_t launch_zeroone_normalize(float* v, int64_t n, float* part, hipStream_t s);
int zeroone_partials_floats();
hipError_t launch_preprocess_video(const uint8_t* frames, int T, int Hs, int Ws, int H, int W, float* out,
                                   hipStream_t s);
hipError_t launch_warp_backward(const float* gout, const float* img, int N, int C, int H, int W, const float* motion,
                                int64_t m_sn, int64_t m_sc, float* gimg, float* gmot, hipStream_t s);
```

### fully-automated-multi-heartbeat-echocardiography-video-segmentation-and-motion-tracking_amd/csrc/plumbing.hip

```cpp
#include <float.h>
#include <stdlib.h>

#include "common.h"

#include "clasfv.h"
#include "plumbing.h"
#include "warp_math.h"

#pragma clang fp contract(off)

namespace {

__device__ inline int round_half_even_div32(int t) {
  const int q = t >> 5, r = t & 31;
  if (r > 16) return q + 1;
  if (r < 16) return q;
  return q + (q & 1);
}

struct Lin {
  int i0, i1;
  float l0, l1;
};

__device__ inline Lin lin_ac_false(int t_in, int t_out, int dst) {
  Lin r;
  const float scale = (float)t_in / (float)t_out;
  float src = fmaf(scale, (float)dst + 0.5f, -0.5f);
  src = fmaxf(src, 0.f);
  r.i0 = min((int)floorf(src), t_in - 1);
  r.l1 = fminf(fmaxf(src - (float)r.i0, 0.f), 1.f);
  r.i1 = r.i0 + (r.i0 < t_in - 1 ? 1 : 0);
  r.l0 = 1.f - r.l1;
  return r;
}

__device__ inline float lerp_t(float a, float b, float l0, float l1) { return fmaf(a, l0, (b * l1)); }

__global__ void build_clips_kernel(const float* __restrict__ video, int T, int HW, const int32_t* __restrict__ table,
                                   int interp, float* __restrict__ clips) {
  const int clip = blockIdx.z, fr = blockIdx.y;
  const int c = fr >> 5, f = fr & 31;
  const int shift = table[2 * clip], j0 = table[2 * clip + 1];
  const int tk = T - shift;
  const int tf = j0 + f;
  const int tc = 32 * round_half_even_div32(tk);
  const float* vc = video + (size_t)c * T * HW;
  float* out = clips + (((size_t)clip * 3 + c) * 32 + f) * HW;
  const bool resample = interp && (tk & 31) && tk != tc;
  Lin L = {0, 0, 1.f, 0.f};
  if (resample) L = lin_ac_false(tk, tc, tf);
  const float* a = vc + (size_t)(shift + (resample ? L.i0 : tf)) * HW;
  const float* b = vc + (size_t)(shift + (resample ? L.i1 : tf)) * HW;
  if ((HW & 3) == 0 && (((uintptr_t)video | (uintptr_t)clips) & 15) == 0) {
    const f32x4* a4 = reinterpret_cast<const f32x4*>(a);
    const f32x4* b4 = reinterpret_cast<const f32x4*>(b);
    f32x4* o4 = reinterpret_cast<f32x4*>(out);
    for (int i = blockIdx.x * blockDim.x + threadIdx.x; i < (HW >> 2); i += gridDim.x * blockDim.x) {
      f32x4 v = a4[i];
      if (resample) {
        const f32x4 w = b4[i];
#pragma unroll
        for (int e = 0; e < 4; ++e) v[e] = lerp_t(v[e], w[e], L.l0, L.l1);
      }
      o4[i] = v;
    }
    return;
  }
  for (int i = blockIdx.x * blockDim.x + threadIdx.x; i < HW; i += gridDim.x * blockDim.x)
    out[i] = resample ? lerp_t(a[i], b[i], L.l0, L.l1) : a[i];
}

struct PassTable {
  int clip0[CLASFV_MAX_PASSES];
};

__device__ inline void softmax2(float x0, float x1, float& p0, float& p1) {
  const float m = fmaxf(x0, x1);
  const float e0 = expf(x0 - m), e1 = expf(x1 - m);
  const float s = e0 + e1;
  p0 = e0 / s;
  p1 = e1 / s;
}

template <bool MARGIN>
__global__ void pass_labels_kernel(const float* __restrict__ logits, PassTable tab, int T, int step, int HW,
                                   int interp, uint8_t* __restrict__ labels) {
  const int k = blockIdx.z, f = blockIdx.y;
  const int tk = T - k * step;
  if (f >= tk) return;
  const int tc = 32 * round_half_even_div32(tk);
  const bool resample = interp && (tk & 31) && tk != tc;
  Lin L = {f, f, 1.f, 0.f};
  if (resample) L = lin_ac_false(tc, tk, f);
  const size_t clip_stride = (size_t)(MARGIN ? 1 : 2) * 32 * HW;
  const float* base = logits + (size_t)tab.clip0[k] * clip_stride;
  const float* a = base + (size_t)(L.i0 >> 5) * clip_stride + (size_t)(L.i0 & 31) * HW;
  const float* b = base + (size_t)(L.i1 >> 5) * clip_stride + (size_t)(L.i1 & 31) * HW;
  const size_t cs = (size_t)32 * HW;
  uint8_t* out = labels + ((size_t)k * T + f) * HW;
  if ((HW & 3) == 0 && ((uintptr_t)logits & 15) == 0 && ((uintptr_t)labels & 3) == 0) {
    auto lab = [&](float xa0, float xa1, float xb0, float xb1) __attribute__((always_inline)) {
      float pa0, pa1;
      softmax2(xa0, xa1, pa0, pa1);
      float q0 = pa0, q1 = pa1;
      if (resample) {
        float pb0, pb1;
        softmax2(xb0, xb1, pb0, pb1);
        q0 = lerp_t(pa0, pb0, L.l0, L.l1);
        q1 = lerp_t(pa1, pb1, L.l0, L.l1);
      }
      return (unsigned)(q1 > q0 ? 1 : 0);
    };
    for (int i = blockIdx.x * blockDim.x + threadIdx.x; i < (HW >> 2); i += gridDim.x * blockDim.x) {
      const f32x4 a0 = reinterpret_cast<const f32x4*>(a)[i];
      const f32x4 a1 = MARGIN ? a0 : reinterpret_cast<const f32x4*>(a + cs)[i];
      f32x4 b0 = a0, b1 = a1;
      if (resample) {
        b0 = reinterpret_cast<const f32x4*>(b)[i];
        b1 = MARGIN ? b0 : reinterpret_cast<const f32x4*>(b + cs)[i];
      }
      unsigned w = 0;
#pragma unroll
      for (int e = 0; e < 4; ++e)
        w |= (MARGIN ? lab(0.f, a0[e], 0.f, b0[e]) : lab(a0[e], a1[e], b0[e], b1[e])) << (8 * e);
      reinterpret_cast<unsigned*>(out)[i] = w;
    }
    return;
  }
  for (int i = blockIdx.x * blockDim.x + threadIdx.x; i < HW; i += gridDim.x * blockDim.x) {
    float pa0, pa1;
    if (MARGIN)
      softmax2(0.f, a[i], pa0, pa1);
    else
      softmax2(a[i], a[i + cs], pa0, pa1);
    float q0 = pa0, q1 = pa1;
    if (resample) {
      float pb0, pb1;
      if (MARGIN)
        softmax2(0.f, b[i], pb0, pb1);
      else
        softmax2(b[i], b[i + cs], pb0, pb1);
      q0 = lerp_t(pa0, pb0, L.l0, L.l1);
      q1 = lerp_t(pa1, pb1, L.l0, L.l1);
    }
    out[i] = q1 > q0 ? 1 : 0;
  }
}

__global__ void logit_margin_kernel(const float* __restrict__ logits, int n, size_t per_clip,
                                    float* __restrict__ margin) {
  if ((((uintptr_t)logits | (uintptr_t)margin) & 15) == 0) {
    const size_t total4 = (size_t)n * per_clip / 4;
    for (size_t g = blockIdx.x * (size_t)blockDim.x + threadIdx.x; g < total4; g += (size_t)gridDim.x * blockDim.x) {
      const size_t e = 4 * g, c = e / per_clip, r = e - c * per_clip;
      const float* l = logits + 2 * c * per_clip + r;
      const f32x4 l0 = *reinterpret_cast<const f32x4*>(l);
      const f32x4 l1 = *reinterpret_cast<const f32x4*>(l + per_clip);
      *reinterpret_cast<f32x4*>(margin + e) = l1 - l0;
    }
    return;
  }
  const size_t total = (size_t)n * per_clip;
  for (size_t e = blockIdx.x * (size_t)blockDim.x + threadIdx.x; e < total; e += (size_t)gridDim.x * blockDim.x) {
    const size_t c = e / per_clip, r = e - c * per_clip;
    const float* l = logits + 2 * c * per_clip + r;
    margin[e] = l[per_clip] - l[0];
  }
}

__device__ inline int n_votes(int i, int K, int step) {
  int nv = 0;
  const int kmax = min(i, K);
  for (int idx = 0; idx < kmax; ++idx) {
    if (i - idx * step < 0) break;
    ++nv;
  }
  return nv;
}

__global__ void fuse_majority_kernel(const uint8_t* __restrict__ labels, int K, int T, int step, int HW,
                                     uint8_t tie_label, uint8_t* __restrict__ fused) {
  const int o = blockIdx.y;
  const int i = o == 0 ? 0 : o + step - 1;
  const int nv = o == 0 ? 1 : n_votes(i, K, step);
  uint8_t* out = fused + (size_t)o * HW;
  for (int p = blockIdx.x * blockDim.x + threadIdx.x; p < HW; p += gridDim.x * blockDim.x) {
    int ones = 0;
    for (int idx = 0; idx < nv; ++idx) ones += labels[((size_t)idx * T + (i - idx * step)) * HW + p];
    out[p] = (nv == 1) ? (uint8_t)ones : 2 * ones == nv ? tie_label : (uint8_t)(2 * ones > nv ? 1 : 0);
  }
}

constexpr int SIMPLE_THREADS = 256;

__device__ inline double block_sum(double v, double* red) {
  for (int off = 32; off > 0; off >>= 1) v += __shfl_xor(v, off, 64);
  const int lane = threadIdx.x & 63, wid = threadIdx.x >> 6;
  __syncthreads();
  if (lane == 0) red[wid] = v;
  __syncthreads();
  double s = 0;
  for (int w = 0; w < SIMPLE_THREADS / 64; ++w) s += red[w];
  return s;
}

__global__ __launch_bounds__(SIMPLE_THREADS) void fuse_simple_kernel(const uint8_t* __restrict__ labels, int K, int T,
                                                                      int step, int HW, uint8_t* __restrict__ fused) {
  extern __shared__ uint8_t est[];
  __shared__ double red[SIMPLE_THREADS / 64];
  __shared__ double wts[CLASFV_MAX_PASSES];
  const int o = blockIdx.x;
  const int i = o == 0 ? 0 : o + step - 1;
  const int nv = o == 0 ? 1 : n_votes(i, K, step);
  uint8_t* out = fused + (size_t)o * HW;
  auto vote = [&](int idx, int p) -> int { return labels[((size_t)idx * T + (i - idx * step)) * HW + p]; };
  if (nv == 1) {
    for (int p = threadIdx.x; p < HW; p += SIMPLE_THREADS) out[p] = (uint8_t)vote(0, p);
    return;
  }
  for (int p = threadIdx.x; p < HW; p += SIMPLE_THREADS) out[p] = 0;
  for (int lab = 1; lab >= 0; --lab) {
    uint64_t keep = (nv >= 64) ? ~0ull : ((1ull << nv) - 1ull);
    for (int idx = 0; idx < nv; ++idx) wts[idx] = 1.0;
    __syncthreads();
    double cnt = 0;
    for (int p = threadIdx.x; p < HW; p += SIMPLE_THREADS) {
      double on = 0, off = 0;
      for (int idx = 0; idx < nv; ++idx) {
        const bool c = vote(idx, p) == lab;
        on += c ? 1.0 : 0.0;
        off += c ? 0.0 : 1.0;
      }
      est[p] = on > off;
      cnt += est[p];
    }
    double conv = block_sum(cnt, red);
    for (int it = 0; it < 25; ++it) {
      double esum = conv;
      double mx = 0;
      for (int idx = 0; idx < nv; ++idx) {
        if (!(keep >> idx & 1ull)) continue;
        double inter = 0, csum = 0;
        for (int p = threadIdx.x; p < HW; p += SIMPLE_THREADS) {
          const bool c = vote(idx, p) == lab;
          csum += c;
          inter += (c && est[p]);
        }
        inter = block_sum(inter, red);
        csum = block_sum(csum, red);
        const double s = csum + esum;
        const double d = (s == 0) ? 1.0 : 2.0 * inter / s;
        const double w = (d + 1.0) * (d + 1.0);
        if (threadIdx.x == 0) wts[idx] = w;
        mx = fmax(mx, w);
      }
      __syncthreads();
      for (int idx = 0; idx < nv; ++idx)
        if ((keep >> idx & 1ull) && !(wts[idx] > 0.05 * mx)) keep &= ~(1ull << idx);
      cnt = 0;
      for (int p = threadIdx.x; p < HW; p += SIMPLE_THREADS) {
        double on = 0, off = 0;
        for (int idx = 0; idx < nv; ++idx) {
          if (!(keep >> idx & 1ull)) continue;
          const bool c = vote(idx, p) == lab;
          if (c)
            on += wts[idx];
          else
            off += wts[idx];
        }
        est[p] = on > off;
        cnt += est[p];
      }
      const double nsum = block_sum(cnt, red);
      const bool stop = fabs(conv - nsum) < 25.0;
      conv = nsum;
      if (stop) break;
    }
    __syncthreads();
    for (int p = threadIdx.x; p < HW; p += SIMPLE_THREADS)
      if (est[p]) out[p] = (uint8_t)lab;
    __syncthreads();
  }
}

constexpr int SIMPLE_FAST_THREADS = 1024;
constexpr int SIMPLE_FAST_MAXV = 16;

template <int N>
__device__ inline void block_sum_vec(const int (&v)[N], int (*red)[2 * SIMPLE_FAST_MAXV + 1], int* tot) {
  const int lane = threadIdx.x & 63, wid = threadIdx.x >> 6;
#pragma unroll
  for (int j = 0; j < N; ++j) {
    int x = v[j];
#pragma unroll
    for (int off = 32; off > 0; off >>= 1) x += __shfl_xor(x, off, 64);
    if (lane == 0) red[wid][j] = x;
  }
  __syncthreads();
  if (threadIdx.x < N) {
    int t = 0;
#pragma unroll
    for (int w = 0; w < SIMPLE_FAST_THREADS / 64; ++w) t += red[w][threadIdx.x];
    tot[threadIdx.x] = t;
  }
  __syncthreads();
}

__global__ __launch_bounds__(SIMPLE_FAST_THREADS) void fuse_simple_fast_kernel(const uint8_t* __restrict__ labels, int K,
                                                                               int T, int step, int HW,
                                                                               uint8_t* __restrict__ fused) {
  constexpr int MV = SIMPLE_FAST_MAXV;
  extern __shared__ uint8_t smem_simple[];
  uint16_t* msk = reinterpret_cast<uint16_t*>(smem_simple);
  uint8_t* est = smem_simple + 2 * (size_t)HW;
  __shared__ int red[SIMPLE_FAST_THREADS / 64][2 * MV + 1];
  __shared__ int tot[2 * MV + 1];
  const int o = blockIdx.x;
  const int i = o == 0 ? 0 : o + step - 1;
  const int nv = o == 0 ? 1 : n_votes(i, K, step);
  uint8_t* out = fused + (size_t)o * HW;
  if (nv == 1) {
    for (int p = threadIdx.x; p < HW; p += SIMPLE_FAST_THREADS) out[p] = labels[(size_t)i * HW + p];
    return;
  }
  const unsigned full = (1u << nv) - 1u;
  for (int p = threadIdx.x; p < HW; p += SIMPLE_FAST_THREADS) {
    unsigned m = 0;
    for (int idx = 0; idx < nv; ++idx) m |= (unsigned)(labels[((size_t)idx * T + (i - idx * step)) * HW + p] != 0) << idx;
    msk[p] = (uint16_t)m;
    est[p] = 0;
  }
  __syncthreads();
  for (int lab = 1; lab >= 0; --lab) {
    unsigned keep = full;
    double wts[MV];
    int inter[MV], csum[MV];
    int conv;
    {
      int acc[2 * MV + 1];
// ... 444 lines not shown
```

### fully-automated-multi-heartbeat-echocardiography-video-segmentation-and-motion-tracking_amd/dist.py

```python
import torch
import torch.distributed as dist

from . import fuse_utils as FU


def shard_bounds(n, rank, world):
    q, r = divmod(n, world)
    lo = rank * q + min(rank, r)
    return lo, lo + q + (1 if rank < r else 0)


def global_clip_plan(video_lengths, num_clips, step, interpolate_last=True):
    plans, off = [], 0
    for t in video_lengths:
        k = FU.clamp_num_clips(t, num_clips, step)
        if k == 0:
            raise IndexError("list index out of range")
        table, clip0 = FU.clip_table(t, k, step, interpolate_last)
        plans.append({"T": t, "K": k, "table": table, "clip0": clip0, "offset": off, "n": len(table)})
        off += len(table)
    return plans, off


def all_gather_clips(local, n_total, rank, world, group=None, force=False):
    if world == 1 and not force:
        return local
    sizes = [shard_bounds(n_total, r, world) for r in range(world)]
    mx = max(hi - lo for lo, hi in sizes)
    pad = torch.zeros((mx,) + tuple(local.shape[1:]), dtype=local.dtype, device=local.device)
    pad[: local.shape[0]] = local
    if dist.get_backend(group) == "gloo":
        bufs = [torch.empty_like(pad) for _ in range(world)]
        dist.all_gather(bufs, pad, group=group)
        out = torch.cat(bufs)
    else:
        out = torch.empty((world * mx,) + tuple(local.shape[1:]), dtype=local.dtype, device=local.device)
        dist.all_gather_into_tensor(out, pad, group=group)
    parts = [out[r * mx: r * mx + (hi - lo)] for r, (lo, hi) in enumerate(sizes)]
    return torch.cat(parts)


def run_clip_shard(n_total, rank, world, compute, empty):
    lo, hi = shard_bounds(n_total, rank, world)
    local = compute(lo, hi) if hi > lo else empty
    return all_gather_clips(local.contiguous(), n_total, rank, world)


def video_owners(plans, world):
    n_total = sum(p["n"] for p in plans)
    blocks = [shard_bounds(n_total, r, world) for r in range(world)]
    owners = []
    for p in plans:
        a, b = p["offset"], p["offset"] + p["n"]
        best, best_n = 0, -1
        for r, (lo, hi) in enumerate(blocks):
            n = max(0, min(b, hi) - max(a, lo))
            if n > best_n:
                best, best_n = r, n
        owners.append(best)
    return owners


def owner_of_clips(plans, world):
    own = []
    for o, p in zip(video_owners(plans, world), plans):
        own.extend([o] * p["n"])
    return own


def exchange_counts(owners, world):
    n_total = len(owners)
    counts = [[0] * world for _ in range(world)]
    for s_ in range(world):
        lo, hi = shard_bounds(n_total, s_, world)
        for g in range(lo, hi):
            counts[s_][owners[g]] += 1
    return counts


def rows_exchanged(owners, world):
    c = exchange_counts(owners, world)
    return sum(c[s_][o] for s_ in range(world) for o in range(world) if s_ != o)


def exchange_to_owners(local, owners, rank, world, group=None, force=False):
    n_total = len(owners)
    counts = exchange_counts(owners, world)
    lo, hi = shard_bounds(n_total, rank, world)
    if not force and (world == 1 or rows_exchanged(owners, world) == 0):
        keep = [g - lo for g in range(lo, hi) if owners[g] == rank]
        if len(keep) == hi - lo:
            return local
        return local[torch.tensor(keep, dtype=torch.long, device=local.device)]
    order = sorted(range(lo, hi), key=lambda g: (owners[g], g))
    send = local[torch.tensor([g - lo for g in order], dtype=torch.long, device=local.device)] if order else local
    send_sizes = counts[rank]
    recv_sizes = [counts[s_][rank] for s_ in range(world)]
    stage = local.is_cuda and dist.get_backend(group) == "gloo"
    dev = "cpu" if stage else local.device
    out = torch.empty((sum(recv_sizes),) + tuple(local.shape[1:]), dtype=local.dtype, device=dev)
    dist.all_to_all_single(out, send.contiguous().to(dev), output_split_sizes=recv_sizes, input_split_sizes=send_sizes,
                           group=group)
    return out.to(local.device) if stage else out


def videos_needed(lengths, num_clips, step, rank, world, interpolate_last=True):
    plans, n_total = global_clip_plan(lengths, num_clips, step, interpolate_last)
    lo, hi = shard_bounds(n_total, rank, world)
    return [vi for vi, p in enumerate(plans) if max(lo, p["offset"]) < min(hi, p["offset"] + p["n"])]


def exchange_stats(lengths, num_clips, step, world, h=112, w=112, interpolate_last=True):
    plans, _ = global_clip_plan(lengths, num_clips, step, interpolate_last)
    rows = rows_exchanged(owner_of_clips(plans, world), world) if world > 1 else 0
    return rows, rows * FU.CLIP * h * w * 4


def segment_videos_sharded(videos_dev, model, num_clips=5, step=1, fuse_method="simple", interpolate_last=True,
                           rank=0, world=1, batch_size=None, clip_fn=None, lengths=None, force_exchange=False,
                           exchange_events=None):
    if lengths is None:
        lengths = [v.shape[1] for v in videos_dev]
    plans, n_total = global_clip_plan(list(lengths), num_clips, step, interpolate_last)
    present = [v for v in videos_dev if v is not None]
    if not present:
        raise ValueError("no video tensor on this rank")
    h, w = present[0].shape[-2:]
    dev = present[0].device

    def compute(lo, hi):
        mine = []
        for vi, p in enumerate(plans):
            a, b = max(lo, p["offset"]), min(hi, p["offset"] + p["n"])
            if a < b:
                if videos_dev[vi] is None:
                    raise ValueError(f"video {vi} has clips in rank {rank}'s block but is not on this rank")
                mine.append(FU.build_clips(videos_dev[vi], p["table"][a - p["offset"]: b - p["offset"]],
                                           interpolate_last))
        clips = torch.cat(mine) if len(mine) > 1 else mine[0]
        return clip_fn(clips) if clip_fn else FU.run_model(model, clips, batch_size)

    empty = torch.empty((0, 2, FU.CLIP, h, w), device=dev, dtype=torch.float32)
    lo, hi = shard_bounds(n_total, rank, world)
    local = compute(lo, hi) if hi > lo else empty
    owners = owner_of_clips(plans, world)
    margin = force_exchange or (world > 1 and rows_exchanged(owners, world) > 0)
    ev = None
    if margin and exchange_events is not None:
        ev = (torch.cuda.Event(enable_timing=True), torch.cuda.Event(enable_timing=True))
        ev[0].record()
    if margin:
        local = FU.logit_margin(local) if local.shape[0] else local[:, 0]
    mine = exchange_to_owners(local.contiguous(), owners, rank, world, force=force_exchange)
    if ev is not None:
        ev[1].record()
        exchange_events.append(ev)
    vown = video_owners(plans, world)
    out, at = {}, 0
    for vi, p in enumerate(plans):
        if vown[vi] != rank:
            continue
        lg = mine[at: at + p["n"]]
        at += p["n"]
        labels = FU.pass_labels(lg, p["clip0"], p["T"], step, interpolate_last, margin=margin)
        out[vi] = FU.fuse_votes(labels, step, fuse_method)
    return out
```

### fully-automated-multi-heartbeat-echocardiography-video-segmentation-and-motion-tracking_amd/fuse_utils.py

```python
import numpy as np
import torch

from . import _lib

FUSE_METHODS = {"majority": _lib.FUSE_MAJORITY, "majorityvoting": _lib.FUSE_MAJORITY, "mv": _lib.FUSE_MAJORITY,
                "itkvoting": _lib.FUSE_ITKVOTING, "voting": _lib.FUSE_ITKVOTING, "simple": _lib.FUSE_SIMPLE,
                "staple": _lib.FUSE_STAPLE}
MAX_PASSES = 64
CLIP = 32
DEFAULT_BATCH = 32


def n_clips(t, clip_length=CLIP):
    return int(np.round(t / clip_length))


def clamp_num_clips(t, num_clips, step, strict_reference=True):
    if t < CLIP + num_clips * step:
        num_clips = (t - CLIP) // step
    if num_clips < 0:
        print("Video is too short")
        num_clips = 1
    if num_clips == 0 and not strict_reference:
        num_clips = 1
    return num_clips


def fused_frames(t, step, strict_reference=True):
    return t if not strict_reference else t - (step - 1)


def keep_dropped_frames(labels, fused, step):
    if step == 1:
        return fused
    return torch.cat([fused[:1], labels[0, 1:step].to(fused.dtype), fused[1:]])


def clip_table(t, num_passes, step, interpolate_last=True):
    table, clip0 = [], []
    for k in range(num_passes):
        shift = k * step
        tk = t - shift
        nk = n_clips(tk)
        if tk % CLIP != 0 and not interpolate_last and nk * CLIP > tk:
            raise ValueError("all the input array dimensions except for the concatenation axis must match exactly")
        if nk == 0:
            raise ValueError(f"pass {k}: {tk} frames give no 32-frame clip")
        clip0.append(len(table))
        table.extend((shift, CLIP * j) for j in range(nk))
    return table, clip0


def _device_of(model):
    eng = getattr(model, "engine", None)
    if eng is not None:
        return eng.device
    return torch.device("cuda", torch.cuda.current_device())


def to_device_video(video, device):
    v = torch.as_tensor(np.asarray(video, np.float32) if not torch.is_tensor(video) else video)
    return v.to(device, torch.float32).contiguous()


_TABLES = {}


def _device_table(table, device):
    key = (str(device), tuple(table))
    t = _TABLES.get(key)
    if t is None:
        if len(_TABLES) > 256:
            _TABLES.clear()
        t = torch.tensor(np.asarray(table, np.int32).reshape(-1), device=device)
        _TABLES[key] = t
    return t


def build_clips(video_dev, table, interpolate_last=True):
    if video_dev.dim() != 4 or video_dev.shape[0] != 3:
        raise ValueError(f"expected a (3,T,H,W) video, got {tuple(video_dev.shape)}")
    video_dev = video_dev.to(torch.float32).contiguous()
    _, t, h, w = video_dev.shape
    tab = _device_table(table, video_dev.device)
    clips = torch.empty((len(table), 3, CLIP, h, w), device=video_dev.device, dtype=torch.float32)
    lib = _lib.load()
    _lib.check(lib.clasfv_build_clips(_lib.ptr(video_dev), t, h, w, _lib.ptr(tab), len(table), int(bool(interpolate_last)),
                                      _lib.ptr(clips), _lib.stream_ptr(device=video_dev.device)), "clasfv_build_clips")
    return clips


def divide_to_consecutive_clips(video, clip_length=CLIP, interpolate_last=False):
    if clip_length != CLIP:
        raise ValueError("the engine uses 32-frame clips")
    dev = torch.device("cuda", torch.cuda.current_device())
    v = to_device_video(video, dev)
    table, _ = clip_table(v.shape[1], 1, 1, interpolate_last)
    return build_clips(v, table, interpolate_last)


def run_model(model, clips, batch_size=None):
    n = clips.shape[0]
    if batch_size is None:
        batch_size = DEFAULT_BATCH if hasattr(model, "engine") else 1
    outs = []
    for s in range(0, n, batch_size):
        seg, _ = model(clips[s:s + batch_size])
        outs.append(seg.to(clips.device, torch.float32))
    return torch.cat(outs) if len(outs) > 1 else outs[0].contiguous()


def fuse_votes(labels, step, fuse_method="simple", force_generic=False):
    labels = labels.to(torch.uint8).contiguous()
    k, t, h, w = labels.shape
    method = FUSE_METHODS.get(fuse_method.lower())
    if method is None:
        raise NotImplementedError(f"fuse_method {fuse_method!r}: supported {sorted(FUSE_METHODS)}")
    if force_generic:
        method |= _lib.FUSE_FORCE_GENERIC
    fused = torch.empty((t - (step - 1), h, w), device=labels.device, dtype=torch.uint8)
    lib = _lib.load()
    _lib.check(lib.clasfv_fuse_votes(_lib.ptr(labels), k, t, step, h, w, method, _lib.ptr(fused),
                                     _lib.stream_ptr(device=labels.device)), "clasfv_fuse_votes")
    return fused


def ctypes_int32_array(vals):
    import ctypes
    arr = (ctypes.c_int32 * max(1, len(vals)))(*vals)
    return ctypes.cast(arr, ctypes.c_void_p), arr


def segment_a_video_with_fusion_device(video, model, interpolate_last=True, step=1, num_clips=10, fuse_method="simple",
                                       class_list=(0, 1), batch_size=None, strict_reference=True):
    if list(class_list) != [0, 1]:
        raise ValueError("the engine fuses the two CLAS-FV classes [0, 1]")
    dev = _device_of(model)
    v = to_device_video(video, dev)
    t = v.shape[1]
    k = clamp_num_clips(t, num_clips, step, strict_reference)
    if k == 0:
        raise IndexError("list index out of range")
    table, clip0 = clip_table(t, k, step, interpolate_last)
    clips = build_clips(v, table, interpolate_last)
    logits = run_model(model, clips, batch_size)
    labels = pass_labels(logits, clip0, t, step, interpolate_last)
    fused = fuse_votes(labels, step, fuse_method)
    return fused if strict_reference else keep_dropped_frames(labels, fused, step)


def logit_margin(logits):
    logits = logits.to(torch.float32).contiguous()
    n, _, c, h, w = logits.shape
    out = torch.empty((n, c, h, w), device=logits.device, dtype=torch.float32)
    lib = _lib.load()
    _lib.check(lib.clasfv_logit_margin(_lib.ptr(logits), n, h, w, _lib.ptr(out), _lib.stream_ptr(device=logits.device)),
               "clasfv_logit_margin")
    return out


def pass_labels(logits, clip0, t, step, interpolate_last=True, margin=False):
    k = len(clip0)
    if k > MAX_PASSES:
        raise ValueError(f"at most {MAX_PASSES} shifted passes are supported (got {k})")
    logits = logits.to(torch.float32).contiguous()
    h, w = logits.shape[-2:]
    labels = torch.empty((k, t, h, w), device=logits.device, dtype=torch.uint8)
    ptr, keep = ctypes_int32_array(clip0)
    lib = _lib.load()
    fn = lib.clasfv_pass_labels_margin if margin else lib.clasfv_pass_labels
    _lib.check(fn(_lib.ptr(logits), k, ptr, t, step, h, w, int(bool(interpolate_last)), _lib.ptr(labels),
                  _lib.stream_ptr(device=logits.device)), "clasfv_pass_labels")
    del keep
    return labels


def segment_a_video_with_fusion(video, model, interpolate_last=True, step=1, num_clips=10, fuse_method="simple",
                                class_list=[0, 1], batch_size=None, strict_reference=True):
    fused = segment_a_video_with_fusion_device(video, model, interpolate_last, step, num_clips, fuse_method, class_list,
                                               batch_size, strict_reference)
    return fused.to(torch.int64).cpu().numpy()
```

### fully-automated-multi-heartbeat-echocardiography-video-segmentation-and-motion-tracking_amd/model.py

```python
import ctypes
import warnings
from collections import OrderedDict

import numpy as np
import torch
from torch import nn

from . import _lib
from .arch import strip_module_prefix
from .weights import DEFAULT_SEED, recipe_state_dict


class Engine:

    def __init__(self, device=None, dtype="fp32"):
        if not torch.cuda.is_available():
            raise RuntimeError("CLAS-FV engine requires a HIP (ROCm) GPU; none is visible")
        self.lib = _lib.load()
        self.device = torch.device("cuda", torch.cuda.current_device() if device is None else
                                   torch.device(device).index or 0)
        h = ctypes.c_void_p()
        _lib.check(self.lib.clasfv_create(self.device.index, ctypes.byref(h)), "clasfv_create")
        self.h = h
        self.set_dtype(dtype)

    def set_dtype(self, dtype):
        if dtype not in _lib.DTYPES:
            raise ValueError(f"dtype must be one of {sorted(_lib.DTYPES)}")
        _lib.check(self.lib.clasfv_set_compute_dtype(self.h, _lib.DTYPES[dtype]), "clasfv_set_compute_dtype")
        self.dtype = "bf16" if _lib.DTYPES[dtype] == 1 else "fp32"

    def set_variants(self, *names):
        flags = 0
        for n in names:
            if n not in _lib.VARIANTS:
                raise ValueError(f"unknown kernel variant {n!r}: {sorted(_lib.VARIANTS)}")
            flags |= _lib.VARIANTS[n]
        old = self.lib.clasfv_get_kernel_variants(self.h)
        _lib.check(self.lib.clasfv_set_kernel_variants(self.h, flags), "clasfv_set_kernel_variants")
        return tuple(n for n, b in _lib.VARIANTS.items() if old & b)

    def __del__(self):
        try:
            if getattr(self, "h", None):
                self.lib.clasfv_destroy(self.h)
                self.h = None
        except Exception:
            pass

    def param_table(self):
        out = []
        name = ctypes.c_char_p()
        nd = ctypes.c_int()
        dims = (ctypes.c_int64 * 5)()
        for i in range(self.lib.clasfv_param_count(self.h)):
            _lib.check(self.lib.clasfv_param_info(self.h, i, ctypes.byref(name), ctypes.byref(nd), dims), "param_info")
            out.append((name.value.decode(), tuple(int(dims[d]) for d in range(nd.value))))
        return out

    def load(self, state):
        for k, v in state.items():
            a = np.ascontiguousarray(np.asarray(v.detach().cpu() if torch.is_tensor(v) else v), dtype=np.float32)
            _lib.check(self.lib.clasfv_load_param(self.h, k.encode(), a.ctypes.data_as(ctypes.c_void_p), a.size),
                       f"load {k}")
        _lib.check(self.lib.clasfv_finalize(self.h), "clasfv_finalize")

    def forward(self, x, seg, mot, stream=None):
        n, c, t, hh, ww = x.shape
        _lib.check(self.lib.clasfv_forward(self.h, _lib.ptr(x), n, t, hh, ww, _lib.ptr(seg), _lib.ptr(mot),
                                           _lib.stream_ptr(stream, self.device)), "clasfv_forward")

    def conv_table(self):
        out = []
        pre, bn = ctypes.c_char_p(), ctypes.c_char_p()
        tap, din, dout = ctypes.c_int(), ctypes.c_int(), ctypes.c_int()
        ch, k, s, p = (ctypes.c_int * 5)(), (ctypes.c_int * 3)(), (ctypes.c_int * 3)(), (ctypes.c_int * 3)()
        for i in range(self.lib.clasfv_conv_count(self.h)):
            _lib.check(self.lib.clasfv_conv_info(self.h, i, ctypes.byref(pre), ctypes.byref(bn), ctypes.byref(tap), ch, k, s,
                                                 p, ctypes.byref(din), ctypes.byref(dout)), "clasfv_conv_info")
            out.append({"index": i, "prefix": pre.value.decode(), "bn": bn.value.decode(), "tap": tap.value,
                        "cin": ch[0], "cout": ch[1], "cin_p": ch[2], "cout_p": ch[3], "cin2": ch[4],
                        "kernel": tuple(k), "stride": tuple(s), "padding": tuple(p),
                        "in_dtype": torch.bfloat16 if din.value == 1 else torch.float32,
                        "out_dtype": torch.bfloat16 if dout.value == 1 else torch.float32})
        return out

    def run_conv(self, i, x, nthw, y, x2=None, res=None, relu=True, x_c8=False, y_c8=False, scratch=None, stream=None):
        name = ctypes.c_char_p()
        n, t, hh, ww = nthw
        opt = lambda a: _lib.ptr(a) if a is not None else None
        _lib.check(self.lib.clasfv_run_conv(self.h, i, _lib.ptr(x), n, t, hh, ww, opt(x2), opt(res), int(bool(relu)),
                                            int(bool(x_c8)), int(bool(y_c8)), _lib.ptr(y), opt(scratch),
                                            scratch.numel() * scratch.element_size() if scratch is not None else 0,
                                            ctypes.byref(name), _lib.stream_ptr(stream, self.device)), "clasfv_run_conv")
        return name.value.decode()

    def run_decoder(self, taps, nthw, seg, mot, stream=None):
        n, t, hh, ww = nthw
        _lib.check(self.lib.clasfv_run_decoder(self.h, *[_lib.ptr(a) for a in taps], n, t, hh, ww, _lib.ptr(seg),
                                               _lib.ptr(mot), _lib.stream_ptr(stream, self.device)), "clasfv_run_decoder")

    def set_launch_log(self, enable=True):
        _lib.check(self.lib.clasfv_set_launch_log(self.h, 1 if enable else 0), "clasfv_set_launch_log")

    def launch_log(self, cap=4096):
        labels = (ctypes.c_char_p * cap)()
        grids = (ctypes.c_int64 * cap)()
        passes = (ctypes.c_int * cap)()
        convs = (ctypes.c_int * cap)()
        n = self.lib.clasfv_launch_log(self.h, cap, labels, grids, passes, convs)
        if n < 0:
            _lib.check(n, "clasfv_launch_log")
        return [(labels[i].decode(), int(grids[i]), int(passes[i]), int(convs[i])) for i in range(n)]

    def set_kernel_timing(self, enable=True):
        _lib.check(self.lib.clasfv_set_kernel_timing(self.h, 1 if enable else 0), "clasfv_set_kernel_timing")

    def kernel_timing(self, cap=16):
        names = (ctypes.c_char_p * cap)()
        launches = (ctypes.c_int * cap)()
        ms = (ctypes.c_double * cap)()
        gf = (ctypes.c_double * cap)()
        xg = (ctypes.c_double * cap)()
        n = self.lib.clasfv_kernel_timing(self.h, cap, names, launches, ms, gf, xg)
        if n < 0:
            _lib.check(n, "clasfv_kernel_timing")
        return {names[i].decode(): {"launches": int(launches[i]), "ms": float(ms[i]), "gflop": float(gf[i]),
                                    "xgflop": float(xg[i])} for i in range(n)}

    def workspace_bytes(self):
        return int(self.lib.clasfv_workspace_bytes(self.h))

    def fill_workspace(self, byte, stream=None):
        _lib.check(self.lib.clasfv_fill_workspace(self.h, int(byte), _lib.stream_ptr(stream, self.device)),
                   "clasfv_fill_workspace")


class R2plus1D_18_MotionNet(nn.Module):

    def __init__(self, pretrained=True, output_channels=4, device=None, seed=DEFAULT_SEED, dtype="fp32",
                 weights="random"):
        super().__init__()
        if output_channels != 4:
            raise ValueError("the motion head has 4 channels [fwd x, fwd y, bwd x, bwd y]")
        if pretrained:
            warnings.warn("pretrained=True: Kinetics weights cannot be downloaded offline; using seeded synthetic "
                          "weights (load a checkpoint with load_state_dict)", stacklevel=2)
        self.engine = Engine(device, dtype)
        self._state = OrderedDict()
        self._params = None
        self._load(recipe_state_dict(weights, seed))

    def set_kernel_variants(self, *names):
        old = self.engine.set_variants(*names)
        self.engine.load(self._state)
        return old

    def set_compute_dtype(self, dtype):
        self.engine.set_dtype(dtype)
        self.engine.load(self._state)
        return self

    def _load(self, sd):
        table = self.engine.param_table()
        state = OrderedDict()
        for name, shape in table:
            if name not in sd:
                raise KeyError(f"missing key in state_dict: {name}")
            v = sd[name]
            t = v.detach().cpu() if torch.is_tensor(v) else torch.from_numpy(np.asarray(v))
            if tuple(t.shape) != shape:
                raise RuntimeError(f"size mismatch for {name}: {tuple(t.shape)} vs {shape}")
            state[name] = t.clone()
        self.engine.load(state)
        self._state = state
        self._params = None

    def load_state_dict(self, state_dict, strict=True):
        sd = OrderedDict((strip_module_prefix(k), v) for k, v in state_dict.items())
        expected = {n for n, _ in self.engine.param_table()}
        unexpected = [k for k in sd if k not in expected]
        missing = [k for k in expected if k not in sd]
        if strict and (unexpected or missing):
            raise RuntimeError(f"Error(s) in loading state_dict: missing={missing[:5]} unexpected={unexpected[:5]}")
        merged = OrderedDict(self._state)
        merged.update({k: v for k, v in sd.items() if k in expected})
        self._load(merged)
        return nn.modules.module._IncompatibleKeys(missing, unexpected)

    def state_dict(self, *args, **kwargs):
        return OrderedDict((k, v.clone()) for k, v in self._state.items())

    def parameters(self, recurse=True):
        if self._params is None:
            self._params = [nn.Parameter(v.float(), requires_grad=True) for k, v in self._state.items()
                            if not k.endswith(("running_mean", "running_var", "num_batches_tracked"))]
        return iter(self._params)

    @torch.no_grad()
    def forward(self, x):
        x = torch.as_tensor(x)
        if x.dim() != 5 or x.shape[1] != 3:
            raise ValueError(f"expected (N,3,T,H,W), got {tuple(x.shape)}")
        x = x.to(self.engine.device, torch.float32).contiguous()
        n, _, t, h, w = x.shape
        seg = torch.empty((n, 2, t, h, w), device=x.device, dtype=torch.float32)
        mot = torch.empty((n, 4, t, h, w), device=x.device, dtype=torch.float32)
        self.engine.forward(x, seg, mot)
        return seg, mot
```

### include/clasfv.h

```cpp
#ifndef CLASFV_H
#define CLASFV_H

#include <stdint.h>

#ifdef __cplusplus
extern "C" {
#endif

enum {
  CLASFV_OK = 0,
  CLASFV_EINVAL = -1,
  CLASFV_EBADSHAPE = -2,
  CLASFV_ENOTREADY = -3,
  CLASFV_EHIP = -4,
  CLASFV_ENOMEM = -5
};

#define CLASFV_ABI_VERSION 3

enum { CLASFV_FUSE_MAJORITY = 0, CLASFV_FUSE_SIMPLE = 1, CLASFV_FUSE_STAPLE = 2, CLASFV_FUSE_ITKVOTING = 3 };
#define CLASFV_FUSE_FORCE_GENERIC 0x100
enum { CLASFV_DTYPE_FP32 = 0, CLASFV_DTYPE_BF16 = 1 };

enum {
  CLASFV_VARIANT_NO_WINOGRAD = 1,
  CLASFV_VARIANT_NO_WINO_PATCH = 2,
  CLASFV_VARIANT_WINOT_REFERENCE = 4,
  CLASFV_VARIANT_NO_C8 = 8,
  CLASFV_VARIANT_NO_STEM_BF16 = 16,
  CLASFV_VARIANT_NO_PATCH_BF16 = 32,
  CLASFV_VARIANT_NO_DECODER_BF16 = 64,
  CLASFV_VARIANT_WINOT_NO_TS1 = 128,
  CLASFV_VARIANT_NO_SPLIT_K = 256,
  CLASFV_VARIANT_NO_WINO4 = 512,
  CLASFV_VARIANT_NO_DECODER_X3 = 1024,
  CLASFV_VARIANT_NO_DMA_X3 = 2048,
  CLASFV_VARIANT_NO_STEM_X3 = 4096,
  CLASFV_VARIANT_NO_WINO4W = 8192,
  CLASFV_VARIANT_NO_PATCH32 = 16384,
  CLASFV_VARIANT_NO_PROJ_X3 = 32768,
  CLASFV_VARIANT_NO_WINO4R = 65536,
  CLASFV_VARIANT_NO_DMA_BUF = 262144,
  CLASFV_VARIANT_W4R_CACHED_STORES = 524288,
  CLASFV_VARIANT_PATCH32_CACHED_STORES = 4194304,
  CLASFV_VARIANT_NO_DMA_W = 16777216,
  CLASFV_VARIANT_NO_TWALK = 67108864
};

typedef struct clasfv_engine* clasfv_t;

const char* clasfv_last_error(void);
int clasfv_version(void);
const char* clasfv_source_hash(void);

int clasfv_create(int device, clasfv_t* out);
int clasfv_destroy(clasfv_t h);
int clasfv_param_count(clasfv_t h);
int clasfv_param_info(clasfv_t h, int i, const char** name, int* ndim, int64_t dims[5]);
int clasfv_load_param(clasfv_t h, const char* name, const float* host_data, int64_t numel);
int clasfv_finalize(clasfv_t h);
int clasfv_forward(clasfv_t h, const float* x_dev, int N, int T, int H, int W, float* seg_dev,
                   float* motion_dev, void* stream);
int64_t clasfv_workspace_bytes(clasfv_t h);
int clasfv_set_compute_dtype(clasfv_t h, int dtype);
int clasfv_get_compute_dtype(clasfv_t h);
int clasfv_set_kernel_variants(clasfv_t h, int flags);
int clasfv_get_kernel_variants(clasfv_t h);

int clasfv_set_kernel_timing(clasfv_t h, int enable);
int clasfv_kernel_timing(clasfv_t h, int cap, const char** names, int* launches, double* ms,
                         double* gflop, double* xgflop);

int clasfv_set_launch_log(clasfv_t h, int enable);
int clasfv_launch_log(clasfv_t h, int cap, const char** labels, int64_t* grids, int* passes, int* convs);
int clasfv_fill_workspace(clasfv_t h, int byte, void* stream);

int clasfv_conv_count(clasfv_t h);
int clasfv_conv_info(clasfv_t h, int i, const char** prefix, const char** bn_prefix, int* tap, int channels[5],
                     int kernel[3], int stride[3], int padding[3], int* in_dtype, int* out_dtype);
int clasfv_run_conv(clasfv_t h, int i, const void* x_dev, int N, int T, int H, int W, const void* x2_dev,
                    const void* res_dev, int relu, int x_c8, int y_c8, void* y_dev, void* scratch_dev,
                    int64_t scratch_bytes, const char** kernel_name, void* stream);
int clasfv_run_decoder(clasfv_t h, const float* p01_dev, const float* p2_dev, const float* p3_dev,
                       const float* p4_dev, int N, int T, int H, int W, float* seg_dev, float* motion_dev,
                       void* stream);

int clasfv_build_clips(const float* video_dev, int T, int H, int W, const int32_t* table_dev, int n,
                       int interpolate, float* clips_dev, void* stream);
int clasfv_pass_labels(const float* logits_dev, int K, const int32_t* pass_clip0, int T, int step, int H,
                       int W, int interpolate, uint8_t* labels_dev, void* stream);
int clasfv_pass_labels_margin(const float* margin_dev, int K, const int32_t* pass_clip0, int T, int step,
                              int H, int W, int interpolate, uint8_t* labels_dev, void* stream);
int clasfv_logit_margin(const float* logits_dev, int n, int H, int W, float* margin_dev, void* stream);
int clasfv_fuse_votes(const uint8_t* labels_dev, int K, int T, int step, int H, int W, int method,
                      uint8_t* fused_dev, void* stream);

int clasfv_warp(const float* img_dev, int N, int C, int H, int W, const float* motion_dev, int64_t m_sn,
                int64_t m_sc, float* out_dev, void* stream);

int clasfv_warp_backward(const float* grad_out_dev, const float* img_dev, int N, int C, int H, int W,
                         const float* motion_dev, int64_t m_sn, int64_t m_sc, float* grad_img_dev,
                         float* grad_motion_dev, void* stream);

#define CLASFV_TRACK_BILINEAR 0
#define CLASFV_TRACK_NEAREST 1
#define CLASFV_TRACK_FORCE_STEPS 0x100
#define CLASFV_TRACK_FORCE_LDS 0x200
#define CLASFV_TRACK_LDS_MAX_PIXELS 20480
#define CLASFV_TRACK_LDS_AUTO_PIXELS 2304
int clasfv_track(const float* img_dev, int N, int C, int H, int W, const float* motion_dev, int64_t m_sn,
                 int64_t m_sc, int64_t m_st, int T, int t0, int t_step, int P, int mode, float* out_dev,
                 void* stream);

#define CLASFV_LV_NPUCKS 10
#define CLASFV_LV_STRIDE 12
#define CLASFV_LV_MAX_PIXELS 162816
int clasfv_lv_geometry(const uint8_t* masks_dev, int64_t F, int H, int W, int label, double sy, double sx,
                       int32_t* area_dev, double* geom_dev, void* stream);

int clasfv_preprocess_video(const uint8_t* frames_dev, int T, int Hs, int Ws, int H, int W, float* out_dev,
                            void* stream);
int64_t clasfv_zeroone_workspace_bytes(void);
int clasfv_zeroone_normalize(float* video_dev, int64_t n_per_channel, float* workspace_dev, void* stream);

#ifdef __cplusplus
}
#endif
#endif
```

Before: 1448.

## Build clips directly into packed NTHW4 layout and skip redundant decoder index fill

```diff
diff --git a/fully-automated-multi-heartbeat-echocardiography-video-segmentation-and-motion-tracking_amd/_lib.py b/fully-automated-multi-heartbeat-echocardiography-video-segmentation-and-motion-tracking_amd/_lib.py
--- a/fully-automated-multi-heartbeat-echocardiography-video-segmentation-and-motion-tracking_amd/_lib.py
+++ b/fully-automated-multi-heartbeat-echocardiography-video-segmentation-and-motion-tracking_amd/_lib.py
@@ -17,6 +17,7 @@
     "clasfv_load_param": (c_int, [_P, c_char_p, _P, c_int64]),
     "clasfv_finalize": (c_int, [_P]),
     "clasfv_forward": (c_int, [_P, _P, c_int, c_int, c_int, c_int, _P, _P, _P]),
+    "clasfv_forward_packed": (c_int, [_P, _P, c_int, c_int, c_int, c_int, _P, _P, _P]),
     "clasfv_workspace_bytes": (c_int64, [_P]),
     "clasfv_set_compute_dtype": (c_int, [_P, c_int]),
     "clasfv_get_compute_dtype": (c_int, [_P]),
@@ -38,6 +39,7 @@
                                 ctypes.POINTER(c_char_p), _P]),
     "clasfv_run_decoder": (c_int, [_P, _P, _P, _P, _P, c_int, c_int, c_int, c_int, _P, _P, _P]),
     "clasfv_build_clips": (c_int, [_P, c_int, c_int, c_int, _P, c_int, c_int, _P, _P]),
+    "clasfv_build_clips_packed": (c_int, [_P, c_int, c_int, c_int, _P, c_int, c_int, _P, _P]),
     "clasfv_pass_labels": (c_int, [_P, c_int, _P, c_int, c_int, c_int, c_int, c_int, _P, _P]),
     "clasfv_pass_labels_margin": (c_int, [_P, c_int, _P, c_int, c_int, c_int, c_int, c_int, _P, _P]),
     "clasfv_logit_margin": (c_int, [_P, c_int, c_int, c_int, _P, _P]),
diff --git a/fully-automated-multi-heartbeat-echocardiography-video-segmentation-and-motion-tracking_amd/build.py b/fully-automated-multi-heartbeat-echocardiography-video-segmentation-and-motion-tracking_amd/build.py
--- a/fully-automated-multi-heartbeat-echocardiography-video-segmentation-and-motion-tracking_amd/build.py
+++ b/fully-automated-multi-heartbeat-echocardiography-video-segmentation-and-motion-tracking_amd/build.py
@@ -11,8 +11,8 @@
 INCLUDE = os.path.join(REPO_DIR, "include")
 LIB_PATH = os.path.join(PKG_DIR, "libclasfv.so")
 SOURCES = ["engine.hip", "conv.hip", "conv_patch.hip", "winograd.hip", "winograd2.hip", "winograd4.hip", "winograd4w.hip",
-           "winograd_t.hip", "decoder.hip", "plumbing.hip", "twalk.hip", "track.hip", "lvgeom.hip"]
-HEADERS = ["common.h", "lvgeom.h", "plumbing.h", "track.h", "warp_math.h", "wino4_common.h"]
+           "winograd_t.hip", "decoder.hip", "plumbing.hip", "clips_packed.hip", "twalk.hip", "track.hip", "lvgeom.hip"]
+HEADERS = ["clip_math.h", "common.h", "lvgeom.h", "plumbing.h", "track.h", "warp_math.h", "wino4_common.h"]
 ARCH = os.environ.get("CLASFV_OFFLOAD_ARCH", "gfx950")
 EXTRA_FLAGS = {"winograd_t.hip": ["-fno-slp-vectorize"]}
 
diff --git a/fully-automated-multi-heartbeat-echocardiography-video-segmentation-and-motion-tracking_amd/csrc/clip_math.h b/fully-automated-multi-heartbeat-echocardiography-video-segmentation-and-motion-tracking_amd/csrc/clip_math.h
--- /dev/null
+++ b/fully-automated-multi-heartbeat-echocardiography-video-segmentation-and-motion-tracking_amd/csrc/clip_math.h
@@ -0,0 +1,28 @@
+#pragma once
+#include <hip/hip_runtime.h>
+
+__device__ inline int round_half_even_div32(int t) {
+  const int q = t >> 5, r = t & 31;
+  if (r > 16) return q + 1;
+  if (r < 16) return q;
+  return q + (q & 1);
+}
+
+struct Lin {
+  int i0, i1;
+  float l0, l1;
+};
+
+__device__ inline Lin lin_ac_false(int t_in, int t_out, int dst) {
+  Lin r;
+  const float scale = (float)t_in / (float)t_out;
+  float src = fmaf(scale, (float)dst + 0.5f, -0.5f);
+  src = fmaxf(src, 0.f);
+  r.i0 = min((int)floorf(src), t_in - 1);
+  r.l1 = fminf(fmaxf(src - (float)r.i0, 0.f), 1.f);
+  r.i1 = r.i0 + (r.i0 < t_in - 1 ? 1 : 0);
+  r.l0 = 1.f - r.l1;
+  return r;
+}
+
+__device__ inline float lerp_t(float a, float b, float l0, float l1) { return fmaf(a, l0, (b * l1)); }
diff --git a/fully-automated-multi-heartbeat-echocardiography-video-segmentation-and-motion-tracking_amd/csrc/clips_packed.hip b/fully-automated-multi-heartbeat-echocardiography-video-segmentation-and-motion-tracking_amd/csrc/clips_packed.hip
--- /dev/null
+++ b/fully-automated-multi-heartbeat-echocardiography-video-segmentation-and-motion-tracking_amd/csrc/clips_packed.hip
@@ -0,0 +1,55 @@
+#include "common.h"
+
+#include "plumbing.h"
+
+#pragma clang fp contract(off)
+#include "clip_math.h"
+
+namespace {
+
+constexpr int PX = 4;
+
+__global__ __launch_bounds__(256) void build_clips_packed_kernel(const float* __restrict__ video, int T, int HW,
+                                          const int32_t* __restrict__ table, int interp, f32x4* __restrict__ xin) {
+  const int clip = blockIdx.z, f = blockIdx.y;
+  const int shift = table[2 * clip], j0 = table[2 * clip + 1];
+  const int tk = T - shift;
+  const int tf = j0 + f;
+  const int tc = 32 * round_half_even_div32(tk);
+  const bool resample = interp && (tk & 31) && tk != tc;
+  Lin L = {0, 0, 1.f, 0.f};
+  if (resample) L = lin_ac_false(tk, tc, tf);
+  const size_t plane = (size_t)T * HW;
+  const float* a = video + (size_t)(shift + (resample ? L.i0 : tf)) * HW;
+  const float* b = video + (size_t)(shift + (resample ? L.i1 : tf)) * HW;
+  f32x4* out = xin + ((size_t)clip * 32 + f) * HW;
+  for (int i0 = blockIdx.x * (256 * PX) + threadIdx.x; i0 < HW; i0 += gridDim.x * (256 * PX)) {
+    f32x4 v[PX], w[PX];
+#pragma unroll
+    for (int u = 0; u < PX; ++u) {
+      const int i = i0 + 256 * u;
+      const int ic = i < HW ? i : i0;
+      v[u] = f32x4{a[ic], a[plane + ic], a[2 * plane + ic], 0.f};
+      if (resample) w[u] = f32x4{b[ic], b[plane + ic], b[2 * plane + ic], 0.f};
+    }
+#pragma unroll
+    for (int u = 0; u < PX; ++u) {
+      if (resample) {
+#pragma unroll
+        for (int c = 0; c < 3; ++c) v[u][c] = lerp_t(v[u][c], w[u][c], L.l0, L.l1);
+      }
+      if (i0 + 256 * u < HW) out[i0 + 256 * u] = v[u];
+    }
+  }
+}
+
+}
+
+hipError_t launch_build_clips_packed(const float* video, int T, int HW, const int32_t* table, int n, int interp,
+                                     float* xin, hipStream_t s) {
+  const int bx = (HW + 256 * PX - 1) / (256 * PX);
+  dim3 grid(bx < 64 ? bx : 64, 32, n);
+  hipLaunchKernelGGL(build_clips_packed_kernel, grid, dim3(256), 0, s, video, T, HW, table, interp,
+                     reinterpret_cast<f32x4*>(xin));
+  return hipGetLastError();
+}
diff --git a/fully-automated-multi-heartbeat-echocardiography-video-segmentation-and-motion-tracking_amd/csrc/common.h b/fully-automated-multi-heartbeat-echocardiography-video-segmentation-and-motion-tracking_amd/csrc/common.h
--- a/fully-automated-multi-heartbeat-echocardiography-video-segmentation-and-motion-tracking_amd/csrc/common.h
+++ b/fully-automated-multi-heartbeat-echocardiography-video-segmentation-and-motion-tracking_amd/csrc/common.h
@@ -142,7 +142,7 @@
 hipError_t launch_twalk_bf16(const ConvParams& p, hipStream_t s);
 bool stem_bf16_supported(const ConvParams& p);
 hipError_t launch_stem_bf16(const ConvParams& p, hipStream_t s);
-hipError_t launch_decoder(const DecParams& p, hipStream_t s);
+hipError_t launch_decoder(const DecParams& p, hipStream_t s, bool fill_index = true);
 constexpr int DECODER_X3_ELEMS = 3 * 4096 + 3 * 1024;
 void decoder_x3_weights(const float* w2, const float* wh, uint16_t* out);
 hipError_t launch_pack_input(const float* x, float* y, int N, int T, int HW, hipStream_t s);
diff --git a/fully-automated-multi-heartbeat-echocardiography-video-segmentation-and-motion-tracking_amd/csrc/decoder.hip b/fully-automated-multi-heartbeat-echocardiography-video-segmentation-and-motion-tracking_amd/csrc/decoder.hip
--- a/fully-automated-multi-heartbeat-echocardiography-video-segmentation-and-motion-tracking_amd/csrc/decoder.hip
+++ b/fully-automated-multi-heartbeat-echocardiography-video-segmentation-and-motion-tracking_amd/csrc/decoder.hip
@@ -515,7 +515,7 @@
 
 }
 
-static hipError_t launch_dec(const DecParams& p, hipStream_t s, int mode, int th = 8) {
+static hipError_t launch_dec(const DecParams& p, hipStream_t s, int mode, int th = 8, bool fill_index = true) {
   if (p.tap[0].T != p.T) return hipErrorInvalidValue;
   for (int i = 0; i < 4; ++i)
     if ((size_t)p.N * p.tap[i].T * p.tap[i].H * p.tap[i].W * 64 >= ((size_t)1 << 31)) return hipErrorInvalidValue;
@@ -543,7 +543,8 @@
   if (!(mode & 16)) {
     if (!p.idx) return hipErrorInvalidValue;
     const int ne = 4 * (p.T + p.H + p.W);
-    CLASFV_LAUNCH(decoder_index_kernel, dim3((unsigned)((ne + 255) / 256)), dim3(256), 0, s, p);
+    if (fill_index)
+      CLASFV_LAUNCH(decoder_index_kernel, dim3((unsigned)((ne + 255) / 256)), dim3(256), 0, s, p);
   }
   CLASFV_LAUNCH(k, dim3((unsigned)nb), dim3(32 * th), lds, s, p);
   return hipGetLastError();
@@ -578,10 +579,10 @@
               3 * 4096 + (((size_t)kb * 16 + l) * 4 + q) * 8 + e, 1024);
 }
 
-hipError_t launch_decoder(const DecParams& p, hipStream_t s) {
+hipError_t launch_decoder(const DecParams& p, hipStream_t s, bool fill_index) {
   if ((p.x3 || p.bf16) && !p.w2x3) return hipErrorInvalidValue;
   const int mode = p.bf16 ? 1 : p.x3 ? 4 : 0;
-  return launch_dec(p, s, mode, 8);
+  return launch_dec(p, s, mode, 8, fill_index);
 }
 
 #ifdef CLASFV_KNOCKOUTS
diff --git a/fully-automated-multi-heartbeat-echocardiography-video-segmentation-and-motion-tracking_amd/csrc/engine.hip b/fully-automated-multi-heartbeat-echocardiography-video-segmentation-and-motion-tracking_amd/csrc/engine.hip
--- a/fully-automated-multi-heartbeat-echocardiography-video-segmentation-and-motion-tracking_amd/csrc/engine.hip
+++ b/fully-automated-multi-heartbeat-echocardiography-video-segmentation-and-motion-tracking_amd/csrc/engine.hip
@@ -206,6 +206,14 @@
     hipStream_t side = nullptr;
     hipEvent_t ev_fork = nullptr, ev_join = nullptr;
     uint64_t last_use = 0;
+    struct IdxKey {
+      const void* at = nullptr;
+      int T = 0, H = 0, W = 0, tap[4][3] = {};
+      bool operator==(const IdxKey& o) const {
+        return at == o.at && T == o.T && H == o.H && W == o.W && !memcmp(tap, o.tap, sizeof tap);
+      }
+    } idx_key;
+    bool idx_valid = false;
   };
   std::vector<Ctx*> ctxs;
   uint64_t ctx_clock = 0;
@@ -848,9 +856,11 @@
         if (c->last_use < cx->last_use) cx = c;
     }
     cx->stream = s;
+    cx->idx_valid = false;
   }
   cx->last_use = ++h->ctx_clock;
   if (bytes > cx->arena_bytes) {
+    cx->idx_valid = false;
     HIP_TRY(hipDeviceSynchronize());
     (void)hipFree(cx->arena);
     cx->arena = nullptr;
@@ -1048,10 +1058,12 @@
 
 int clasfv_get_kernel_variants(clasfv_t h) { return h ? h->tune.vflags : CLASFV_EINVAL; }
 
-int clasfv_forward(clasfv_t h, const float* x, int N, int T, int H, int W, float* seg, float* mot, void* stream) {
+static int forward_impl(clasfv_t h, const float* x, bool packed, int N, int T, int H, int W, float* seg, float* mot,
+                        void* stream) {
   if (!h) return fail(CLASFV_EINVAL, "null handle");
   if (!h->ready) return fail(CLASFV_ENOTREADY, "clasfv_finalize has not been called");
   if (!x || !seg || !mot) return fail(CLASFV_EINVAL, "null tensor");
+  if (packed && ((uintptr_t)x & 15)) return fail(CLASFV_EINVAL, "packed input must be 16-byte aligned");
   if (N < 1) return fail(CLASFV_EINVAL, "N must be >= 1");
   if (T < 8 || H < 16 || W < 16 || T % 8 || H % 16 || W % 16)
     return fail(CLASFV_EBADSHAPE, "shape must satisfy T % 8 == 0, H % 16 == 0, W % 16 == 0 (got T=" +
@@ -1064,6 +1076,8 @@
   if (int rc_ = acquire_ctx(h, s, L.total, &cx)) return rc_;
   char* const arena = cx->arena;
   auto buf = [&](int b) { return reinterpret_cast<void*>(arena + L.off[b]); };
+  const bool idx_was_valid = cx->idx_valid;
+  cx->idx_valid = false;
   int last_ev = h->ktime ? tick(h, s) : -1;
   auto timed = [&](const char* name, double gflop, double xgflop) {
     if (last_ev < 0) return;
@@ -1123,16 +1137,20 @@
     return rc_;
   };
 
-  log_begin(h);
-  HIP_TRY(launch_pack_input(x, reinterpret_cast<float*>(buf(XIN)), N, T, H * W, s));
-  log_end(h, -1);
-  timed("pack_input_kernel", 0.0, 0.0);
+  const void* xin = x;
+  if (!packed) {
+    log_begin(h);
+    HIP_TRY(launch_pack_input(x, reinterpret_cast<float*>(buf(XIN)), N, T, H * W, s));
+    log_end(h, -1);
+    timed("pack_input_kernel", 0.0, 0.0);
+    xin = buf(XIN);
+  }
   Shape5 sx{N, T, H, W, 4}, s0, sx0;
   Shape5 sp, sp2, sp3, sp4;
   int rc;
   size_t ci = 0;
   const int c8s = c8_pair(h->convs[0], h->convs[1], sx, h->tune);
-  if ((rc = run(h->convs[ci++], buf(XIN), sx, buf(S0), s0, nullptr, true, nullptr, 0, c8s))) return rc;
+  if ((rc = run(h->convs[ci++], xin, sx, buf(S0), s0, nullptr, true, nullptr, 0, c8s))) return rc;
   if ((rc = run(h->convs[ci++], buf(S0), s0, buf(X0), sx0, nullptr, true, nullptr, c8s, 0))) return rc;
   const int outs[4][2] = {{L1A, L1}, {L2A, L2}, {L3A, L3}, {L4A, L4}};
   void* cur = buf(X0);
@@ -1179,13 +1197,28 @@
   const float* tp[4];
   for (int i = 0; i < 4; ++i) tp[i] = reinterpret_cast<const float*>(buf(tb[i]));
   const DecParams d = decoder_params(h, tp, tsh, seg, mot, N, T, H, W, buf(DIDX));
+  clasfv_engine::Ctx::IdxKey key;
+  key.at = d.idx, key.T = T, key.H = H, key.W = W;
+  for (int i = 0; i < 4; ++i) key.tap[i][0] = tsh[i].t, key.tap[i][1] = tsh[i].h, key.tap[i][2] = tsh[i].w;
+  const bool fill_idx = !(idx_was_valid && key == cx->idx_key);
   log_begin(h);
-  HIP_TRY(launch_decoder(d, s));
+  HIP_TRY(launch_decoder(d, s, fill_idx));
   log_end(h, -1);
+  cx->idx_key = key;
+  cx->idx_valid = true;
   const double dec_px = d.x3 ? 6.0 * (64 * 64 + 64 * 16) : d.bf16 ? 3.0 * 64 * 64 + 6.0 * 64 * 16 : 64 * 64 + 64 * 16;
   timed(d.x3 || d.bf16 ? "decoder_kernel" : "decoder_kernel_f32", 2.0 * N * (double)T * H * W * (64 * 64 + 64 * 6) * 1e-9,
         2.0 * N * (double)T * H * W * dec_px * 1e-9);
   return CLASFV_OK;
+}
+
+int clasfv_forward(clasfv_t h, const float* x, int N, int T, int H, int W, float* seg, float* mot, void* stream) {
+  return forward_impl(h, x, false, N, T, H, W, seg, mot, stream);
+}
+
+int clasfv_forward_packed(clasfv_t h, const float* xin, int N, int T, int H, int W, float* seg, float* mot,
+                          void* stream) {
+  return forward_impl(h, xin, true, N, T, H, W, seg, mot, stream);
 }
 
 int clasfv_set_kernel_timing(clasfv_t h, int enable) {
@@ -1255,6 +1288,7 @@
     if (c->stream == s) cx = c;
   if (!cx || !cx->arena) return fail(CLASFV_EINVAL, "no workspace exists for this stream yet");
   DEVICE_GUARD(h->device);
+  cx->idx_valid = false;
   HIP_TRY(hipMemsetAsync(cx->arena, byte, cx->arena_bytes, s));
   return CLASFV_OK;
 }
@@ -1328,6 +1362,7 @@
     if (k) t = half(t), hh = half(hh), ww = half(ww);
     tsh[k] = Shape5{N, t, hh, ww, 64};
   }
+  cx->idx_valid = false;
   log_begin(h);
   HIP_TRY(launch_decoder(decoder_params(h, taps, tsh, seg, mot, N, T, H, W, cx->arena + L.off[DIDX]), s));
   log_end(h, -1);
@@ -1339,6 +1374,15 @@
   if (!video || !table || !clips || n < 0 || T < 1 || H < 1 || W < 1) return fail(CLASFV_EINVAL, "bad argument");
   if (n == 0) return CLASFV_OK;
   HIP_TRY(launch_build_clips(video, T, H * W, table, n, interp, clips, (hipStream_t)stream));
+  return CLASFV_OK;
+}
+
+int clasfv_build_clips_packed(const float* video, int T, int H, int W, const int32_t* table, int n, int interp,
+                              float* xin, void* stream) {
+  if (!video || !table || !xin || n < 0 || T < 1 || H < 1 || W < 1) return fail(CLASFV_EINVAL, "bad argument");
+  if ((uintptr_t)xin & 15) return fail(CLASFV_EINVAL, "packed clips must be 16-byte aligned");
+  if (n == 0) return CLASFV_OK;
+  HIP_TRY(launch_build_clips_packed(video, T, H * W, table, n, interp, xin, (hipStream_t)stream));
   return CLASFV_OK;
 }
 
diff --git a/fully-automated-multi-heartbeat-echocardiography-video-segmentation-and-motion-tracking_amd/csrc/plumbing.h b/fully-automated-multi-heartbeat-echocardiography-video-segmentation-and-motion-tracking_amd/csrc/plumbing.h
--- a/fully-automated-multi-heartbeat-echocardiography-video-segmentation-and-motion-tracking_amd/csrc/plumbing.h
+++ b/fully-automated-multi-heartbeat-echocardiography-video-segmentation-and-motion-tracking_amd/csrc/plumbing.h
@@ -7,6 +7,8 @@
 
 hipError_t launch_build_clips(const float* video, int T, int HW, const int32_t* table, int n, int interp, float* clips,
                               hipStream_t s);
+hipError_t launch_build_clips_packed(const float* video, int T, int HW, const int32_t* table, int n, int interp,
+                                     float* xin, hipStream_t s);
 hipError_t launch_pass_labels(const float* logits, int K, const int32_t* clip0, int T, int step, int HW, int interp,
                               int margin, uint8_t* labels, hipStream_t s);
 hipError_t launch_logit_margin(const float* logits, int n, int HW, float* margin, hipStream_t s);
diff --git a/fully-automated-multi-heartbeat-echocardiography-video-segmentation-and-motion-tracking_amd/csrc/plumbing.hip b/fully-automated-multi-heartbeat-echocardiography-video-segmentation-and-motion-tracking_amd/csrc/plumbing.hip
--- a/fully-automated-multi-heartbeat-echocardiography-video-segmentation-and-motion-tracking_amd/csrc/plumbing.hip
+++ b/fully-automated-multi-heartbeat-echocardiography-video-segmentation-and-motion-tracking_amd/csrc/plumbing.hip
@@ -9,33 +9,9 @@
 
 #pragma clang fp contract(off)
 
+#include "clip_math.h"
+
 namespace {
-
-__device__ inline int round_half_even_div32(int t) {
-  const int q = t >> 5, r = t & 31;
-  if (r > 16) return q + 1;
-  if (r < 16) return q;
-  return q + (q & 1);
-}
-
-struct Lin {
-  int i0, i1;
-  float l0, l1;
-};
-
-__device__ inline Lin lin_ac_false(int t_in, int t_out, int dst) {
-  Lin r;
-  const float scale = (float)t_in / (float)t_out;
-  float src = fmaf(scale, (float)dst + 0.5f, -0.5f);
-  src = fmaxf(src, 0.f);
-  r.i0 = min((int)floorf(src), t_in - 1);
-  r.l1 = fminf(fmaxf(src - (float)r.i0, 0.f), 1.f);
-  r.i1 = r.i0 + (r.i0 < t_in - 1 ? 1 : 0);
-  r.l0 = 1.f - r.l1;
-  return r;
-}
-
-__device__ inline float lerp_t(float a, float b, float l0, float l1) { return fmaf(a, l0, (b * l1)); }
 
 __global__ void build_clips_kernel(const float* __restrict__ video, int T, int HW, const int32_t* __restrict__ table,
                                    int interp, float* __restrict__ clips) {
diff --git a/fully-automated-multi-heartbeat-echocardiography-video-segmentation-and-motion-tracking_amd/dist.py b/fully-automated-multi-heartbeat-echocardiography-video-segmentation-and-motion-tracking_amd/dist.py
--- a/fully-automated-multi-heartbeat-echocardiography-video-segmentation-and-motion-tracking_amd/dist.py
+++ b/fully-automated-multi-heartbeat-echocardiography-video-segmentation-and-motion-tracking_amd/dist.py
@@ -135,8 +135,12 @@
             if a < b:
                 if videos_dev[vi] is None:
                     raise ValueError(f"video {vi} has clips in rank {rank}'s block but is not on this rank")
-                mine.append(FU.build_clips(videos_dev[vi], p["table"][a - p["offset"]: b - p["offset"]],
-                                           interpolate_last))
+                mine.append((videos_dev[vi], p["table"][a - p["offset"]: b - p["offset"]]))
+        if not clip_fn and FU.takes_packed(model):
+            mine = [(v.to(torch.float32).contiguous(), table) for v, table in mine]
+            return FU.run_model_packed(model, mine, interpolate_last,
+                                       batch_size if batch_size is not None else FU.DEFAULT_BATCH)
+        mine = [FU.build_clips(v, table, interpolate_last) for v, table in mine]
         clips = torch.cat(mine) if len(mine) > 1 else mine[0]
         return clip_fn(clips) if clip_fn else FU.run_model(model, clips, batch_size)
 
diff --git a/fully-automated-multi-heartbeat-echocardiography-video-segmentation-and-motion-tracking_amd/fuse_utils.py b/fully-automated-multi-heartbeat-echocardiography-video-segmentation-and-motion-tracking_amd/fuse_utils.py
--- a/fully-automated-multi-heartbeat-echocardiography-video-segmentation-and-motion-tracking_amd/fuse_utils.py
+++ b/fully-automated-multi-heartbeat-echocardiography-video-segmentation-and-motion-tracking_amd/fuse_utils.py
@@ -90,6 +90,48 @@
     return clips
 
 
+def build_clips_packed(video_dev, table, interpolate_last=True, out=None):
+    if video_dev.dim() != 4 or video_dev.shape[0] != 3:
+        raise ValueError(f"expected a (3,T,H,W) video, got {tuple(video_dev.shape)}")
+    video_dev = video_dev.to(torch.float32).contiguous()
+    _, t, h, w = video_dev.shape
+    tab = _device_table(table, video_dev.device)
+    if out is None:
+        out = torch.empty((len(table), CLIP, h, w, 4), device=video_dev.device, dtype=torch.float32)
+    elif tuple(out.shape) != (len(table), CLIP, h, w, 4) or out.dtype != torch.float32 or not out.is_contiguous():
+        raise ValueError(f"out must be a contiguous float32 {(len(table), CLIP, h, w, 4)}")
+    lib = _lib.load()
+    _lib.check(lib.clasfv_build_clips_packed(_lib.ptr(video_dev), t, h, w, _lib.ptr(tab), len(table),
+                                             int(bool(interpolate_last)), _lib.ptr(out),
+                                             _lib.stream_ptr(device=video_dev.device)), "clasfv_build_clips_packed")
+    return out
+
+
+def takes_packed(model):
+    return hasattr(model, "engine") and hasattr(model, "forward_packed")
+
+
+def run_model_packed(model, segments, interpolate_last=True, batch_size=None):
+    if batch_size is None:
+        batch_size = DEFAULT_BATCH
+    flat = [(v, row) for v, table in segments for row in table]
+    outs = []
+    for s in range(0, len(flat), batch_size):
+        rows = flat[s:s + batch_size]
+        _, _, h, w = rows[0][0].shape
+        xin = torch.empty((len(rows), CLIP, h, w, 4), device=rows[0][0].device, dtype=torch.float32)
+        a = 0
+        while a < len(rows):
+            b = a
+            while b < len(rows) and rows[b][0] is rows[a][0]:
+                b += 1
+            build_clips_packed(rows[a][0], [r for _, r in rows[a:b]], interpolate_last, out=xin[a:b])
+            a = b
+        seg, _ = model.forward_packed(xin)
+        outs.append(seg)
+    return torch.cat(outs) if len(outs) > 1 else outs[0]
+
+
 def divide_to_consecutive_clips(video, clip_length=CLIP, interpolate_last=False):
     if clip_length != CLIP:
         raise ValueError("the engine uses 32-frame clips")
@@ -132,7 +174,7 @@
 
 
 def segment_a_video_with_fusion_device(video, model, interpolate_last=True, step=1, num_clips=10, fuse_method="simple",
-                                       class_list=(0, 1), batch_size=None, strict_reference=True):
+                                       class_list=(0, 1), batch_size=None, strict_reference=True, packed=None):
     if list(class_list) != [0, 1]:
         raise ValueError("the engine fuses the two CLAS-FV classes [0, 1]")
     dev = _device_of(model)
@@ -142,8 +184,10 @@
     if k == 0:
         raise IndexError("list index out of range")
     table, clip0 = clip_table(t, k, step, interpolate_last)
-    clips = build_clips(v, table, interpolate_last)
-    logits = run_model(model, clips, batch_size)
+    if takes_packed(model) if packed is None else packed:
+        logits = run_model_packed(model, [(v, table)], interpolate_last, batch_size)
+    else:
+        logits = run_model(model, build_clips(v, table, interpolate_last), batch_size)
     labels = pass_labels(logits, clip0, t, step, interpolate_last)
     fused = fuse_votes(labels, step, fuse_method)
     return fused if strict_reference else keep_dropped_frames(labels, fused, step)
diff --git a/fully-automated-multi-heartbeat-echocardiography-video-segmentation-and-motion-tracking_amd/model.py b/fully-automated-multi-heartbeat-echocardiography-video-segmentation-and-motion-tracking_amd/model.py
--- a/fully-automated-multi-heartbeat-echocardiography-video-segmentation-and-motion-tracking_amd/model.py
+++ b/fully-automated-multi-heartbeat-echocardiography-video-segmentation-and-motion-tracking_amd/model.py
@@ -69,6 +69,11 @@
         n, c, t, hh, ww = x.shape
         _lib.check(self.lib.clasfv_forward(self.h, _lib.ptr(x), n, t, hh, ww, _lib.ptr(seg), _lib.ptr(mot),
                                            _lib.stream_ptr(stream, self.device)), "clasfv_forward")
+
+    def forward_packed(self, xin, seg, mot, stream=None):
+        n, t, hh, ww, _ = xin.shape
+        _lib.check(self.lib.clasfv_forward_packed(self.h, _lib.ptr(xin), n, t, hh, ww, _lib.ptr(seg), _lib.ptr(mot),
+                                                  _lib.stream_ptr(stream, self.device)), "clasfv_forward_packed")
 
     def conv_table(self):
         out = []
@@ -208,3 +213,15 @@
         mot = torch.empty((n, 4, t, h, w), device=x.device, dtype=torch.float32)
         self.engine.forward(x, seg, mot)
         return seg, mot
+
+    @torch.no_grad()
+    def forward_packed(self, xin):
+        if xin.dim() != 5 or xin.shape[4] != 4 or xin.dtype != torch.float32 or xin.device != self.engine.device:
+            raise ValueError(f"expected (N,T,H,W,4) float32 on {self.engine.device}, got {tuple(xin.shape)} {xin.dtype} "
+                             f"on {xin.device}")
+        xin = xin.contiguous()
+        n, t, h, w, _ = xin.shape
+        seg = torch.empty((n, 2, t, h, w), device=xin.device, dtype=torch.float32)
+        mot = torch.empty((n, 4, t, h, w), device=xin.device, dtype=torch.float32)
+        self.engine.forward_packed(xin, seg, mot)
+        return seg, mot
diff --git a/include/clasfv.h b/include/clasfv.h
--- a/include/clasfv.h
+++ b/include/clasfv.h
@@ -61,6 +61,8 @@
 int clasfv_finalize(clasfv_t h);
 int clasfv_forward(clasfv_t h, const float* x_dev, int N, int T, int H, int W, float* seg_dev,
                    float* motion_dev, void* stream);
+int clasfv_forward_packed(clasfv_t h, const float* xin_dev, int N, int T, int H, int W, float* seg_dev,
+                          float* motion_dev, void* stream);
 int64_t clasfv_workspace_bytes(clasfv_t h);
 int clasfv_set_compute_dtype(clasfv_t h, int dtype);
 int clasfv_get_compute_dtype(clasfv_t h);
@@ -87,6 +89,8 @@
 
 int clasfv_build_clips(const float* video_dev, int T, int H, int W, const int32_t* table_dev, int n,
                        int interpolate, float* clips_dev, void* stream);
+int clasfv_build_clips_packed(const float* video_dev, int T, int H, int W, const int32_t* table_dev, int n,
+                              int interpolate, float* xin_dev, void* stream);
 int clasfv_pass_labels(const float* logits_dev, int K, const int32_t* pass_clip0, int T, int step, int H,
                        int W, int interpolate, uint8_t* labels_dev, void* stream);
 int clasfv_pass_labels_margin(const float* margin_dev, int K, const int32_t* pass_clip0, int T, int step,
```

Result: no change. 1459 (median of 6 runs) (+0.7%).
